# haesungpyun/seoul_tourism_recommendation_NGCF

Hardware: NVIDIA B200
Metric: ngcf_epoch_time_fwd_bwd_bpr (lower is better)
Workload: dtype f32

## Files before the change

### include/ngcf_b200.h

```cpp
#ifndef NGCF_B200_H
#define NGCF_B200_H

#include <stddef.h>
#include <stdint.h>

#ifdef __cplusplus
extern "C" {
#endif

#define NGCF_B200_ABI_VERSION 4
#define NGCF_MAX_LAYERS 8
#define NGCF_MAX_WIDTH 128
#define NGCF_ADAM_MAX_TENSORS 32

typedef enum {
    NGCF_OK = 0,
    NGCF_ERR_INVALID = -1,
    NGCF_ERR_CUDA = -2,
    NGCF_ERR_WORKSPACE = -3
} ngcf_status;

int ngcf_abi_version(void);
const char* ngcf_last_error(void);
uint64_t ngcf_launch_count(void);

int ngcf_coo_to_csr_workspace(int64_t nnz, int64_t n_rows, size_t* bytes_host);
int ngcf_coo_to_csr(const int64_t* coo_row, const int64_t* coo_col, int64_t nnz,
                    int64_t n_rows, int64_t n_cols, int transpose,
                    int32_t* rowptr ,
                    int32_t* colidx , int32_t* perm ,
                    void* workspace, size_t workspace_bytes, void* stream);

typedef struct ngcf_csr {
    int64_t n_rows;
    const int32_t* rowptr;
    const int32_t* ent;
    const int32_t* tiles;
    const int32_t* hub_of_row;
    const int32_t* hub_chunk_ptr;
    const int32_t* chunk_ptr;
    const int32_t* hub_ent;
    const int32_t* chunk_row;
    const int32_t* chunk_tiles;
    const int32_t* hub_rows;
    int32_t* hub_done;
    const uint32_t* key_l;
    const uint32_t* key_t;
    int64_t key_row_offset;
    int32_t n_tiles, n_hub, n_chunks, n_chunk_tiles;
    int32_t rowptr_nnz;
    const uint32_t* tile_hubmask;
} ngcf_csr;

int ngcf_spmm_split_threshold(void);
int ngcf_spmm_tile_rows(void);
int ngcf_spmm_tile_entries(void);

int ngcf_edge_entries(const int32_t* colidx, const float* coo_val, const int32_t* perm, const uint8_t* keep_mask,
                      int32_t* ent_out, int64_t nnz, void* stream);

int ngcf_feature_mix(float* user_w, int64_t n_user, int d,
                     const float* const* tables_host, const int* widths_host,
                     const int64_t* const* idx_host, const int64_t* u_id, int64_t batch,
                     float ratio, int32_t* winner, void* stream);

int ngcf_spmm(const ngcf_csr* csr_host, const float* X, int64_t ldx, int d,
              const float* addend, int64_t ld_add,
              const int32_t* slot, const float* gsum, int64_t ld_gsum,
              float* hub_partial,
              float drop_p, uint64_t seed, const uint64_t* seed_dev, int layer, int transposed, int64_t row_offset,
              const uint8_t* keep_bits, const int32_t* c_ent, const int32_t* c_cnt,
              float* Y, int64_t ldy, void* stream);

int ngcf_node_dropout_bits(const ngcf_csr* csr_host, float drop_p, uint64_t seed, const uint64_t* seed_dev,
                           int n_layers, int64_t row_offset, uint8_t* bits_as_L, uint8_t* bits_as_Lt, void* stream);

int ngcf_node_dropout_compact(const ngcf_csr* csr_host, float drop_p, uint64_t seed, const uint64_t* seed_dev,
                              int n_layers, int64_t row_offset,
                              int32_t* const* ent_as_L_host, int32_t* const* cnt_as_L_host,
                              int32_t* const* ent_as_Lt_host, int32_t* const* cnt_as_Lt_host, void* stream);

int ngcf_entry_keys(const ngcf_csr* csr_host, int64_t row_offset, uint32_t* key_l, uint32_t* key_t, void* stream);

int ngcf_plgraph_entries(int64_t n_user, int64_t n_item, int64_t n_edges, double alpha, uint64_t seed,
                         int64_t row0, int64_t n_rows, unsigned long long* total_dev,
                         unsigned long long* keys_or_null, int64_t capacity, void* stream);
int ngcf_build_tiles(const int32_t* rowptr, int64_t n_rows, int max_rows, int max_ent, int32_t* next_scratch,
                     int32_t* tiles_out, int64_t capacity, int32_t* count_out, void* stream);

int ngcf_exchange_flag_words(void);
int ngcf_push_rows(float* const* matrix_on_rank_host, uint32_t* const* flags_on_rank_host, uint32_t* local_state,
                   int world, int rank, int64_t row0, int64_t n_rows, int d, float* multicast_or_null, void* stream);
int ngcf_push_selected_rows(float* const* matrix_on_rank_host, uint32_t* const* flags_on_rank_host, uint32_t* local_state,
                            int world, int rank, int64_t row0, int64_t n_rows, int d,
                            const int64_t* const* lists_host, const int64_t* list_offsets_host,
                            const int64_t* list_sizes_host, int n_lists, float* multicast_or_null, void* stream);

int ngcf_pack_weights(const float* W1, const float* b1, const float* W2, const float* b2,
                      int d_in, int d_out, float* wcat , float* bias_eff ,
                      void* stream);
int ngcf_pack_weights_all(const float* const* W1_host, const float* const* b1_host, const float* const* W2_host,
                          const float* const* b2_host, const int* d_in_host, const int* d_out_host, int n_layers,
                          float* const* wcat_host, float* const* bias_host, void* stream);
int ngcf_dense_fwd(const float* S, const float* E, int64_t n_rows, int d_in, int d_out,
                   const float* wcat, const float* bias_eff, float slope,
                   const float* mess_mult, const uint32_t* mess_bits, float mess_p, uint64_t seed,
                   const uint64_t* seed_dev, int layer, int64_t row_offset, float* E_out, void* stream);

int ngcf_mess_dropout_bits(int64_t n_rows, int d_out, float mess_p, uint64_t seed, const uint64_t* seed_dev, int layer,
                           int64_t row_offset, uint32_t* bits, void* stream);

int ngcf_gather_concat(const float* const* layers_host, const int* dims_host, int n_layers_plus1,
                       const int64_t* rows, int64_t row_offset, int64_t n_out,
                       float* out, int64_t ld_out, void* stream);
int ngcf_gather_concat_sets(const float* const* layers_host, const int* dims_host, int n_layers_plus1,
                            const int64_t* const* rows_host, const int64_t* offsets_host, const int64_t* sizes_host,
                            float* const* outs_host, int n_sets, int64_t ld_out, void* stream);

int ngcf_bpr_fwd_bwd(const float* u, const float* p, const float* n, int64_t batch, int D,
                     float weight_decay, float batch_size_ctor, float reg_w_u, float reg_w_p, float reg_w_n,
                     float* loss, float* gu, float* gp, float* gn, void* stream);

int ngcf_rowgrad_scatter(const int64_t* const* rows_host, const int64_t* offsets_host,
                         const float* const* g_host, const int64_t* batch_host, int n_sets, int D,
                         int32_t* slot, float* gsum, void* stream);
int ngcf_rowgrad_normalize(const int64_t* const* rows_host, const int64_t* offsets_host,
                           const int64_t* batch_host, int n_sets, const float* const* layers_host,
                           const int* dims_host, int n_layers_plus1, const int32_t* slot, float* gsum, int D,
                           void* stream);
int ngcf_rowgrad_reset(const int64_t* const* rows_host, const int64_t* offsets_host,
                       const int64_t* batch_host, int n_sets, int32_t* slot, void* stream);

int ngcf_set_wgrad_stream(void* stream_or_null);
int ngcf_wgrad_stream_forked(void);
int ngcf_dense_bwd(const float* gE_next, const int32_t* slot, const float* gsum, int64_t ld_gsum, int col_off,
                   const float* E_out, const float* S, const float* E, int64_t n_rows, int d_in, int d_out,
                   const float* W1, const float* W2, float slope,
                   const float* mess_mult, const uint32_t* mess_bits, float mess_p, uint64_t seed,
                   const uint64_t* seed_dev, int layer, int64_t row_offset, int gh_normalized, float* gS, float* gEl,
                   float* gW1, float* gb1, float* gW2, float* gb2, float* gM_scratch, void* stream);

int ngcf_score_topk_workspace(int64_t n_users, int64_t n_items, int D, int k, size_t* bytes_host);
int ngcf_score_topk(const float* U, int64_t n_users, const float* I, int64_t n_items, int D, int k,
                    float* out_val , int64_t* out_idx ,
                    void* workspace, size_t workspace_bytes, void* stream);
int ngcf_score_topk_excluding(const float* U, int64_t n_users, const float* I, int64_t n_items, int D, int k,
                              const int64_t* excl_ptr , const int32_t* excl_idx,
                              float* out_val , int64_t* out_idx ,
                              void* workspace, size_t workspace_bytes, void* stream);

int ngcf_rank_metrics(const int64_t* topk_idx, int64_t n_users, int k, const int64_t* truth_ptr,
                      const int32_t* truth_idx, const int* Ks_host, int n_K, float* per_user, float* totals,
                      void* stream);

int ngcf_adam_step(float* const* params_host, float* const* grads_host, float* const* exp_avg_host,
                   float* const* exp_avg_sq_host, const int64_t* sizes_host, int n_tensors, double lr, double beta1,
                   double beta2, double eps, double weight_decay, int64_t step, const int64_t* step_dev,
                   int zero_grads, void* stream);

int ngcf_eval_groups(const float* u, const float* items, const int64_t* item_ids, const float* rating,
                     const int64_t* group_ptr, int64_t n_groups, int group, int D, int k_hr, int k_ndcg, float weight_decay,
                     float batch_size_ctor, float* bpr, float* hit, float* ndcg, float* rmse, float* scores,
                     float* totals, void* stream);

int ngcf_sample_negatives(const int32_t* pos_ptr, const int32_t* pos_idx, const int64_t* row_user, int64_t n_rows,
                          const int64_t* candidates, int n_candidates, int ng_ratio, uint64_t seed, int64_t* out,
                          int32_t* n_short, void* stream);

int ngcf_laplacian_entries(const int64_t* user, const int64_t* item, const float* rating, int64_t n_pairs,
                           int64_t n_user, int64_t n_item, int32_t* deg, int64_t* row, int64_t* col, float* val,
                           void* stream);

int ngcf_debug_bwd_timeline(int enable, long long* out_host);
int ngcf_debug_spmm_timeline(unsigned long long* dev_buf_or_null);
int ngcf_debug_compact_timeline(unsigned long long* dev_buf_or_null);

#ifdef __cplusplus
}
#endif
#endif
```

### seoul_tourism_recommendation_ngcf_b200/NGCF.py

```python
from __future__ import annotations

import ctypes as C
import os

import numpy as np
import torch
import torch.nn as nn

import torch.distributed as dist

from . import _lib
from .plan import LaplacianPlan, node_dropout_bits, node_dropout_compact, spmm
from .sharded import RowShards, all_gather_rows

LEAKY_SLOPE = 0.2


def _stream() -> int:
    return _lib.current_stream()


class _Ctx:
    __slots__ = ("plan", "E", "S", "dims", "vals_f", "vals_b", "mess_mult", "mess_p", "seed", "seed_dev", "masked", "drop_p", "bits_f", "bits_b", "comp_f", "comp_b", "mess_bits",
                 "rows", "offsets", "W1", "W2", "fresh_key", "node_mode", "last_partial", "fm_stream")


def _capturing() -> bool:
    return torch.cuda.is_current_stream_capturing()


def _join_feature_mix(st):
    if st.fm_stream is not None:
        torch.cuda.current_stream().wait_stream(st.fm_stream)
        st.fm_stream = None


class _Propagate(torch.autograd.Function):

    @staticmethod
    def forward(ctx, mod, st: _Ctx, n_sets, user_w, item_w, *wb):
        lib = _lib.load()
        K = mod.n_layer
        W1, b1, W2, b2 = wb[0:K], wb[K:2 * K], wb[2 * K:3 * K], wb[3 * K:4 * K]
        dev = user_w.device
        sh = mod._shard
        N = mod.n_user + mod.n_item
        r0, nloc, nv = (sh.r0, sh.rows, sh.valid) if sh is not None else (0, N, N)
        X0 = mod._packed_table()
        if mod._snapshot:
            _join_feature_mix(st)
            X0 = X0.clone()
        st.E, st.S, st.W1, st.W2 = [X0], [], list(W1), list(W2)
        side = st.plan.fwd
        st.bits_f = st.bits_b = st.comp_f = st.comp_b = None
        st.node_mode = mod._node_mode
        st.last_partial = None
        if st.drop_p > 0:
            shared = st.plan.side(True, False) is side
            node_mode = mod._node_mode if all(d % 4 == 0 for d in st.dims) or mod._node_mode == "inkernel" else "bits"
            st.node_mode = node_mode
            if node_mode == "compact":
                st.comp_f, ct = node_dropout_compact(side, st.drop_p, st.seed, st.seed_dev, K, r0, as_L=True, as_Lt=shared)
                if shared:
                    st.comp_b = ct
            elif node_mode == "bits":
                st.bits_f, bt = node_dropout_bits(side, st.drop_p, st.seed, st.seed_dev, K, r0, as_L=True, as_Lt=shared)
                if shared:
                    st.bits_b = bt
        self_uses_mess_bits = mod._mess_bits
        st.mess_bits = [None] * K
        for k in range(K):
            if self_uses_mess_bits and st.mess_mult is None and st.mess_p[k] > 0 and st.dims[k + 1] % 4 == 0:
                bits = torch.empty(nloc * ((st.dims[k + 1] + 31) // 32), dtype=torch.int32, device=dev)
                _lib.check(lib.ngcf_mess_dropout_bits(nv, st.dims[k + 1], float(st.mess_p[k]), st.seed,
                                                      _lib.ptr(st.seed_dev), k, r0, bits.data_ptr(), _stream()),
                           "mess_dropout_bits")
                st.mess_bits[k] = bits
        wcats = [torch.empty(2 * st.dims[k] * st.dims[k + 1], dtype=torch.float32, device=dev) for k in range(K)]
        biases = [torch.empty(st.dims[k + 1], dtype=torch.float32, device=dev) for k in range(K)]
        _lib.check(lib.ngcf_pack_weights_all(_lib.ptr_array(W1), _lib.ptr_array(b1), _lib.ptr_array(W2), _lib.ptr_array(b2),
                                             _lib.int_array(st.dims[:K]), _lib.int_array(st.dims[1:]), K,
                                             _lib.ptr_array(wcats), _lib.ptr_array(biases), _stream()), "pack_weights_all")
        _join_feature_mix(st)
        for k in range(K):
            d_in, d_out = st.dims[k], st.dims[k + 1]
            vals = st.vals_f[k] if st.vals_f is not None else None
            S = spmm(side, vals, st.E[k], d_in, drop_p=st.drop_p, seed=st.seed, seed_dev=st.seed_dev, layer=k,
                     row_offset=r0, keep_bits=st.bits_f,
                     compact=st.comp_f[k] if st.comp_f is not None else None)
            wcat, bias = wcats[k], biases[k]
            xkey = None
            if sh is None:
                Xn = En = torch.empty(N, d_out, dtype=torch.float32, device=dev)
            elif mod._xchg is not None and d_out % 4 == 0:
                xkey = ("E", k + 1)
                Xn = mod._xchg.matrix(xkey, sh.N_pad, d_out)
                En = Xn[r0:r0 + nloc]
            else:
                Xn = torch.empty(sh.N_pad, d_out, dtype=torch.float32, device=dev)
                En = torch.zeros(nloc, d_out, dtype=torch.float32, device=dev) if nv < nloc else \
                    torch.empty(nloc, d_out, dtype=torch.float32, device=dev)
            mm = st.mess_mult[k] if st.mess_mult is not None else None
            E_loc = st.E[k][r0:r0 + nloc]
            _lib.check(lib.ngcf_dense_fwd(S.data_ptr(), E_loc.data_ptr(), nv, d_in, d_out, wcat.data_ptr(),
                                          bias.data_ptr(), LEAKY_SLOPE, _lib.ptr(mm[r0:r0 + nloc] if mm is not None else None),
                                          _lib.ptr(st.mess_bits[k]), float(st.mess_p[k]), st.seed, _lib.ptr(st.seed_dev), k, r0, En.data_ptr(),
                                          _stream()),
                       "dense_fwd")
            if xkey is not None and k == K - 1:
                mod._xchg.push_selected(xkey, r0, nloc, st.rows[:n_sets], st.offsets[:n_sets])
                st.last_partial = xkey
            elif xkey is not None:
                mod._xchg.push(xkey, r0, nloc)
            elif sh is not None:
                all_gather_rows(Xn, En, mod._group)
            st.S.append(S)
            st.E.append(Xn)
        D = sum(st.dims)
        layers, dims = _lib.ptr_array(st.E), _lib.int_array(st.dims)
        outs = [torch.empty(st.rows[j].numel(), D, dtype=torch.float32, device=dev) for j in range(n_sets)]
        _lib.check(lib.ngcf_gather_concat_sets(layers, dims, K + 1, _lib.ptr_array(st.rows[:n_sets]),
                                               _lib.i64_array(st.offsets[:n_sets]),
                                               _lib.i64_array([r.numel() for r in st.rows[:n_sets]]), _lib.ptr_array(outs),
                                               n_sets, D, _stream()), "gather_concat_sets")
        ctx.st, ctx.mod, ctx.n_sets = st, mod, n_sets
        return tuple(outs)

    @staticmethod
    def backward(ctx, *gouts):
        lib = _lib.load()
        st, mod, n_sets = ctx.st, ctx.mod, ctx.n_sets
        mod._check_fresh(st, "loss.backward()")
        K, dims = mod.n_layer, st.dims
        dev = st.E[0].device
        sh = mod._shard
        N = mod.n_user + mod.n_item
        r0, nloc, nv, N_all = (sh.r0, sh.rows, sh.valid, sh.N_pad) if sh is not None else (0, N, N, N)
        D = sum(dims)
        g = [(go.contiguous() if go is not None else torch.zeros(st.rows[j].numel(), D, device=dev))
             for j, go in enumerate(gouts)]
        batch = [r.numel() for r in st.rows[:n_sets]]
        rows_h, offs_h = _lib.ptr_array(st.rows[:n_sets]), _lib.i64_array(st.offsets[:n_sets])
        g_h, batch_h = _lib.ptr_array(g), _lib.i64_array(batch)
        slot = mod._slot_map(N_all, dev)
        gsum = torch.empty(sum(batch), D, dtype=torch.float32, device=dev)
        _lib.check(lib.ngcf_rowgrad_scatter(rows_h, offs_h, g_h, batch_h, n_sets, D, slot.data_ptr(),
                                            gsum.data_ptr(), _stream()), "rowgrad_scatter")
        _lib.check(lib.ngcf_rowgrad_normalize(rows_h, offs_h, batch_h, n_sets, _lib.ptr_array(st.E), _lib.int_array(dims),
                                              K + 1, slot.data_ptr(), gsum.data_ptr(), D, _stream()), "rowgrad_normalize")
        slot_loc = slot[r0:r0 + nloc]
        sizes = [dims[k + 1] * dims[k] for k in range(K)]
        n_flat = 2 * sum(sizes) + 2 * sum(dims[1:])
        if sh is not None and mod._xchg is not None:
            f_pad = (n_flat + 3) // 4 * 4
            wg_all = mod._xchg.matrix(("wgrad", f_pad), sh.world, f_pad)
            flat = wg_all[sh.rank, :n_flat]
            flat.zero_()
        else:
            wg_all = None
            flat = torch.zeros(n_flat, dtype=torch.float32, device=dev)
        gW1, gW2, gb1, gb2, o = [], [], [], [], 0
        for k in range(K):
            gW1.append(flat[o:o + sizes[k]].view(dims[k + 1], dims[k])); o += sizes[k]
            gW2.append(flat[o:o + sizes[k]].view(dims[k + 1], dims[k])); o += sizes[k]
            gb1.append(flat[o:o + dims[k + 1]]); o += dims[k + 1]
            gb2.append(flat[o:o + dims[k + 1]]); o += dims[k + 1]
        side = st.plan.side(True, st.vals_b is not None)
        if st.drop_p > 0 and st.node_mode == "compact" and st.comp_b is None:
            _, st.comp_b = node_dropout_compact(side, st.drop_p, st.seed, st.seed_dev, K, r0, as_L=False, as_Lt=True)
        if st.drop_p > 0 and st.node_mode == "bits" and st.bits_b is None:
            _, st.bits_b = node_dropout_bits(side, st.drop_p, st.seed, st.seed_dev, K, r0, as_L=False, as_Lt=True)
        gE_next = None
        col_off = D
        overlap = _capturing() or (sh is not None and mod._xchg is not None)
        if overlap:
            if mod._side_stream is None:
                mod._side_stream = torch.cuda.Stream(device=dev)
            _lib.check(lib.ngcf_set_wgrad_stream(mod._side_stream.cuda_stream), "set_wgrad_stream")
            lib.ngcf_wgrad_stream_forked()
            gM_keep = []
        else:
            gM_scratch = torch.empty(nloc, max(dims[1:]), dtype=torch.float32, device=dev)
        for k in range(K - 1, -1, -1):
            d_in, d_out = dims[k], dims[k + 1]
            col_off -= d_out
            peer = sh is not None and mod._xchg is not None and d_in % 4 == 0
            if peer:
                gS_all = mod._xchg.matrix(("gS", d_in), N_all, d_in)
                gS = gS_all[r0:r0 + nloc]
            else:
                gS = torch.empty(nloc, d_in, dtype=torch.float32, device=dev)
            if peer and k == 0:
                gE0_all = mod._xchg.matrix(("gE0", d_in), N_all, d_in)
                gEl = gE0_all[r0:r0 + nloc]
            else:
                gEl = torch.empty(nloc, d_in, dtype=torch.float32, device=dev)
            mm = st.mess_mult[k] if st.mess_mult is not None else None
            if overlap:
                gM_scratch = torch.empty(nloc, dims[k + 1], dtype=torch.float32, device=dev)
                gM_keep.append(gM_scratch)
            _lib.check(lib.ngcf_dense_bwd(_lib.ptr(gE_next), slot_loc.data_ptr(), gsum.data_ptr(), D, col_off,
                                          st.E[k + 1][r0:r0 + nloc].data_ptr(), st.S[k].data_ptr(),
                                          st.E[k][r0:r0 + nloc].data_ptr(), nv, d_in, d_out,
                                          st.W1[k].data_ptr(), st.W2[k].data_ptr(), LEAKY_SLOPE,
                                          _lib.ptr(mm[r0:r0 + nloc] if mm is not None else None),
                                          _lib.ptr(st.mess_bits[k]), float(st.mess_p[k]), st.seed,
                                          _lib.ptr(st.seed_dev), k, r0, 1, gS.data_ptr(),
                                          gEl.data_ptr(),
                                          gW1[k].data_ptr(), gb1[k].data_ptr(), gW2[k].data_ptr(), gb2[k].data_ptr(),
                                          gM_scratch.data_ptr(), _stream()), "dense_bwd")
            if peer:
                mod._xchg.push(("gS", d_in), r0, nloc)
            elif sh is not None:
                gS_all = torch.empty(N_all, d_in, dtype=torch.float32, device=dev)
                all_gather_rows(gS_all, gS, mod._group)
            else:
                gS_all = gS
            vals = st.vals_b[k] if st.vals_b is not None else None
            last = (k == 0)
            gE_next = spmm(side, vals, gS_all, d_in, addend=gEl, slot=slot_loc if last else None,
                           gsum=gsum if last else None, drop_p=st.drop_p, seed=st.seed, seed_dev=st.seed_dev, layer=k,
                           transposed=True, row_offset=r0, keep_bits=st.bits_b,
                           compact=st.comp_b[k] if st.comp_b is not None else None)
            if mod._trace is not None:
                mod._trace.append(dict(k=k, gS=gS.clone(), gEl=gEl.clone(), gE=gE_next.clone()))
        if overlap:
            _lib.check(lib.ngcf_set_wgrad_stream(None), "set_wgrad_stream")
            if lib.ngcf_wgrad_stream_forked():
                torch.cuda.current_stream().wait_stream(mod._side_stream)
        _lib.check(lib.ngcf_rowgrad_reset(rows_h, offs_h, batch_h, n_sets, slot.data_ptr(), _stream()),
                   "rowgrad_reset")
        if sh is not None:
            if mod._xchg is not None and dims[0] % 4 == 0:
                mod._xchg.push(("gE0", dims[0]), r0, nloc)
                gE0 = gE0_all.clone()
            else:
                gE0 = torch.empty(N_all, dims[0], dtype=torch.float32, device=dev)
                all_gather_rows(gE0, gE_next, mod._group)
            if wg_all is not None:
                mod._xchg.push(("wgrad", wg_all.shape[1]), sh.rank, 1)
                total = wg_all.sum(0)[:n_flat]
                gW1, gW2, gb1, gb2, o = [], [], [], [], 0
                for k in range(K):
                    gW1.append(total[o:o + sizes[k]].view(dims[k + 1], dims[k])); o += sizes[k]
                    gW2.append(total[o:o + sizes[k]].view(dims[k + 1], dims[k])); o += sizes[k]
                    gb1.append(total[o:o + dims[k + 1]]); o += dims[k + 1]
                    gb2.append(total[o:o + dims[k + 1]]); o += dims[k + 1]
            else:
                dist.all_reduce(flat, group=mod._group)
        else:
            gE0 = gE_next
        gU, gI = gE0[:mod.n_user], gE0[mod.n_user:N]
        return (None, None, None, gU, gI, *gW1, *gb1, *gW2, *gb2)


class NGCF(nn.Module):

    def __init__(self, embed_size: int, layer_size: list, node_dropout: float, mess_dropout: list,
                 emb_ratio: float, lap_list: list, num_dict: dict, batch_size: int, device, *, rng: str = "device",
                 snapshot: bool = False):
        super().__init__()
        if rng not in ("device", "reference"):
            raise ValueError("rng must be 'device' or 'reference'")
        self.n_user = int(num_dict['user'])
        self.n_item = int(num_dict['item'])
        self.emb_size = int(embed_size)
        self.weight_size = list(layer_size)
        self.n_layer = len(self.weight_size)
        self.batch_size = batch_size
        self.device = device
        self.node_dropout = node_dropout
        self.mess_dropout = mess_dropout
        self.emb_ratio = emb_ratio
        self.rng = rng
        if max([self.emb_size] + self.weight_size) > 128 or self.n_layer > 8:
            raise ValueError("embedding/layer widths up to 128 and up to 8 layers are supported")

        w = self.emb_size // 5
        self.feat_widths = [w, w, w, w, self.emb_size - 4 * w]
        self.month_emb = nn.Embedding(int(num_dict['month']), w)
        self.day_emb = nn.Embedding(int(num_dict['day']), w)
        self.sex_emb = nn.Embedding(int(num_dict['sex']), w)
        self.age_emb = nn.Embedding(int(num_dict['age']), w)
        self.dow_emb = nn.Embedding(int(num_dict['dayofweek']), self.feat_widths[4])
        self.item_embedding = nn.Embedding(self.n_item, self.emb_size)
        self.user_embedding = nn.Embedding(self.n_user, self.emb_size)
        self.lap_list = lap_list
        self.set_layers()
        self._plans = {}
        self._table = None
        self._slot = None
        self._winner = None
        self._last = None
        self._all_E = None
        self._mess_bits = os.environ.get("NGCF_B200_MESS_BITS", "0") == "1"
        self._node_mode = "compact"
        self._snapshot = bool(snapshot) or os.environ.get("NGCF_B200_SNAPSHOT", "0") == "1"
        self._mix_count = 0
        self._seed_gen = None
        self._seed_dev = None
        self._shard = None
        self._group = None
        self._xchg = None
        self._side_stream = None
        self._side_stream3 = None
        self._trace = None
        self._inject = None

    def set_layers(self):
        init = nn.init.kaiming_uniform_
        init(self.user_embedding.weight)
        init(self.item_embedding.weight)
        init(self.age_emb.weight)
        init(self.sex_emb.weight)
        init(self.month_emb.weight)
        init(self.dow_emb.weight)
        init(self.day_emb.weight)
        sizes = [self.emb_size] + self.weight_size
        w1, w2, nd, md = [], [], [], []
        for k in range(self.n_layer):
            w1.append(nn.Linear(sizes[k], sizes[k + 1], bias=True))
            w2.append(nn.Linear(sizes[k], sizes[k + 1], bias=True))
            if self.node_dropout is not None:
                nd.append(nn.Dropout(p=self.node_dropout))
            if self.mess_dropout is not None:
                md.append(nn.Dropout(p=self.mess_dropout[k]))
        self.w1_list = nn.Sequential(*w1)
        self.w2_list = nn.Sequential(*w2)
        self.node_dropout_list = nn.Sequential(*nd)
        self.mess_dropout_list = nn.Sequential(*md)

    def shard(self, group=None, shards=None):
        if not dist.is_initialized():
            raise RuntimeError("NGCF.shard() needs an initialised torch.distributed process group")
        if self.rng != "device":
            raise ValueError("row-sharded runs need rng='device' (masks are keyed on global coordinates in-kernel)")
        world, rank = dist.get_world_size(group), dist.get_rank(group)
        self._shard = shards if shards is not None else RowShards(self.n_user + self.n_item, world, rank)
        if self._shard.N != self.n_user + self.n_item or self._shard.world != world or self._shard.rank != rank:
            raise ValueError("the shard descriptor does not match this model / process group")
        self._group = group
        self._plans, self._table, self._slot = {}, None, None
        self._xchg = None
        if world > 1 and os.environ.get("NGCF_B200_EXCHANGE", "peer") != "nccl":
            try:
                from .sharded import PeerExchange
                self._xchg = PeerExchange(group, self.user_embedding.weight.device)
            except Exception as e:
                self._xchg_error = f"{type(e).__name__}: {e}"
                ok = torch.tensor([0], device=self.user_embedding.weight.device)
            else:
                ok = torch.tensor([1], device=self.user_embedding.weight.device)
            dist.all_reduce(ok, op=dist.ReduceOp.MIN, group=group)
            if int(ok) == 0:
                self._xchg = None
        if self._xchg is None and world > 1 and not getattr(self._shard, "equal", True):
            raise RuntimeError("unequal row blocks (BalancedShards) need the peer-memory exchange, which is not available "
                               "here: " + getattr(self, "_xchg_error", "disabled by NGCF_B200_EXCHANGE=nccl"))
        return self

    def exchange_description(self) -> str:
        if self._shard is None:
            return "single GPU"
        if self._xchg is not None:
            how = "NVLS multicast stores (multimem.st)" if self._xchg.multicast() else "peer-memory stores"
            return (f"contiguous row blocks; per-layer exchange of E / gS / table-gradient rows by {how} over NVLink "
                    "(ngcf_push_rows on symmetric memory, no NCCL collective anywhere in the step; the last layer's "
                    "output travels for the batch rows only; W/b gradients: one more push + a rank-ordered sum)")
        return "equal row blocks, per-layer NCCL all-gather of E / gS, all-reduce of W/b grads"

    def _packed_table(self) -> torch.Tensor:
        u, i = self.user_embedding.weight, self.item_embedding.weight
        d = self.emb_size
        adjacent = (u.is_contiguous() and i.is_contiguous() and u.dtype == torch.float32 and
                    u.data_ptr() + self.n_user * d * 4 == i.data_ptr() and
                    getattr(self, "_table", None) is not None and self._table.data_ptr() == u.data_ptr())
        if not adjacent:
            n_rows = self._shard.N_pad if self._shard is not None else self.n_user + self.n_item
            table = torch.zeros(n_rows, d, dtype=torch.float32, device=u.device)
            table[:self.n_user].copy_(u.data)
            table[self.n_user:self.n_user + self.n_item].copy_(i.data)
            u.data = table[:self.n_user]
            i.data = table[self.n_user:self.n_user + self.n_item]
            self._table = table
        return self._table if self._shard is None else self._table

    def _slot_map(self, N, dev):
        if self._slot is None or self._slot.device != dev or self._slot.numel() != N:
            self._slot = torch.full((N,), -1, dtype=torch.int32, device=dev)
        return self._slot

    def _plan(self, year_idx: int, dev) -> LaplacianPlan:
        L = self.lap_list[year_idx]
        p = self._plans.get(year_idx)
        if p is None or p.src is not L or p.coo_val.device != dev:
            p = LaplacianPlan(L, dev, shard=self._shard)
            self._plans[year_idx] = p
        return p

    def _reference_node_masks(self, nnz: int, dev):
        alive = np.arange(nnz)
        out = []
        for _ in range(self.n_layer):
            m = nn.Dropout(self.node_dropout)(torch.tensor(np.ones(alive.size))).type(torch.bool).numpy()
            alive = alive[m]
            full = np.zeros(nnz, dtype=np.uint8)
            full[alive] = 1
            out.append(torch.from_numpy(full).to(dev))
        return out

    @_lib.on_device
    def forward(self, year, u_id, age, sex, month, day, dow, pos_item, neg_item, node_flag):
        lib = _lib.load()
        dev = self.user_embedding.weight.device
        if dev.type != "cuda":
            raise RuntimeError("NGCF (B200) runs on a CUDA device only; there is no CPU fallback. "
                               "Move the module with .to('cuda').")
        K, N = self.n_layer, self.n_user + self.n_item
        if (self._side_stream is None or self._side_stream.device != dev) and not _capturing():
            self._side_stream, self._side_stream3 = (torch.cuda.Stream(device=dev) for _ in range(2))

        def ix(t):
            return t.to(device=dev, dtype=torch.int64).contiguous()

        u_id, pos_item = ix(u_id), ix(pos_item)
        feats_idx = [ix(age), ix(sex), ix(month), ix(day), ix(dow)]
        has_neg = len(neg_item) > 0
        neg_item = ix(neg_item) if has_neg else None
        year_idx = int(year.min()) % 18

        table = self._packed_table()
        if self._winner is None or self._winner.device != dev or self._winner.numel() != self.n_user:
            self._winner = torch.full((self.n_user,), -1, dtype=torch.int32, device=dev)
        tabs = [self.age_emb.weight, self.sex_emb.weight, self.month_emb.weight, self.day_emb.weight, self.dow_emb.weight]
        def mix():
            _lib.check(lib.ngcf_feature_mix(table.data_ptr(), self.n_user, self.emb_size, _lib.ptr_array(tabs),
                                            _lib.int_array(self.feat_widths), _lib.ptr_array(feats_idx), u_id.data_ptr(),
                                            u_id.numel(), float(self.emb_ratio), self._winner.data_ptr(), _stream()),
                       "feature_mix")

        fm_stream = None
        if self._shard is None and _capturing() and bool(node_flag) and \
                (self.node_dropout or 0) > 0 and self.rng == "device":
            main = torch.cuda.current_stream()
            if self._side_stream3 is None:
                self._side_stream3 = torch.cuda.Stream(device=dev)
            self._side_stream3.wait_stream(main)
            with torch.cuda.stream(self._side_stream3):
                mix()
            fm_stream = self._side_stream3
        else:
            mix()

        self._mix_count += 1
        st = _Ctx()
        st.fm_stream = fm_stream
        st.fresh_key = self._fresh_key()
        st.plan = plan = self._plan(year_idx, dev)
        if self._shard is not None and "edge_keep" in (self._inject or {}):
            raise ValueError("explicit edge masks are not supported in row-sharded mode")
        if plan.N != N:
            raise ValueError(f"Laplacian is {plan.N}x{plan.N} but n_user+n_item = {N}")
        st.dims = [self.emb_size] + self.weight_size
        inj = self._inject or {}
        st.masked = bool(node_flag) and (self.node_dropout is not None) and \
            (self.node_dropout > 0 or "edge_keep" in inj)
        st.vals_f = st.vals_b = None
        st.drop_p = 0.0
        masks = None
        if st.masked:
            if "edge_keep" in inj:
                masks = [m.to(device=dev, dtype=torch.uint8).contiguous() for m in inj["edge_keep"]]
            elif self.rng == "reference":
                masks = self._reference_node_masks(plan.nnz, dev)
            else:
                st.drop_p = float(self.node_dropout)
        st.mess_mult = None
        st.mess_p = [0.0] * K
        if "mess_mult" in inj:
            st.mess_mult = [m.to(device=dev, dtype=torch.float32).contiguous() for m in inj["mess_mult"]]
        elif self.training and self.mess_dropout is not None:
            st.mess_p = [float(p) for p in self.mess_dropout[:K]]
        need_seed = st.drop_p > 0 or any(p > 0 for p in st.mess_p)
        if not need_seed:
            st.seed = 0
        elif self.rng == "reference":
            if self._seed_gen is None:
                self._seed_gen = torch.Generator().manual_seed(torch.initial_seed() & (2 ** 63 - 1))
            st.seed = int(torch.randint(0, 2 ** 62, (1,), generator=self._seed_gen).item())
        else:
            st.seed = int(torch.randint(0, 2 ** 62, (1,)).item())
        st.seed_dev = self._seed_dev if need_seed else None
        if masks is not None:
            st.vals_f = [plan.entries(plan.fwd, masks[k]) for k in range(K)]
            st.vals_b = [plan.entries(plan.bwd, masks[k]) for k in range(K)]
        st.rows = [u_id, pos_item] + ([neg_item] if has_neg else [])
        st.offsets = [0, self.n_user] + ([self.n_user] if has_neg else [])

        wb = [l.weight for l in self.w1_list] + [l.bias for l in self.w1_list] + \
             [l.weight for l in self.w2_list] + [l.bias for l in self.w2_list]
        outs = _Propagate.apply(self, st, len(st.rows), self.user_embedding.weight, self.item_embedding.weight, *wb)
        self._last, self._all_E = st, None
        u_embeddings, pos_i_embeddings = outs[0], outs[1]
        neg_i_embeddings = outs[2] if has_neg else torch.empty(0)
        return u_embeddings, pos_i_embeddings, neg_i_embeddings

    def _fresh_key(self):
        return (self._mix_count, _lib.param_epoch(), self.user_embedding.weight._version,
                self.item_embedding.weight._version)

    def _check_fresh(self, st, what: str):
        if self._snapshot or st.fresh_key == self._fresh_key():
            return
        why = "the step that produced it also ran the optimizer" if st.fresh_key is None else \
            "another forward (feature mix) or an optimizer step ran since"
        raise RuntimeError(f"NGCF (B200): {what} needs the embedding table as the forward left it, but {why}. "
                           "Run the forward again, or construct the module with snapshot=True to keep a per-forward "
                           "copy like the reference's torch.cat (NGCF.py:120).")

    @_lib.on_device
    def _materialize(self):
        if self._last is None:
            raise AttributeError("all_users_emb / all_items_emb exist after the first forward (NGCF.py:148-149)")
        if self._all_E is None:
            self._check_fresh(self._last, "all_users_emb / all_items_emb")
            if self._last.last_partial is not None:
                sh = self._shard
                self._xchg.push(self._last.last_partial, sh.r0, sh.rows)
                self._last.last_partial = None
            st, lib = self._last, _lib.load()
            N, D = self.n_user + self.n_item, sum(st.dims)
            out = torch.empty(N, D, dtype=torch.float32, device=st.E[0].device)
            _lib.check(lib.ngcf_gather_concat(_lib.ptr_array(st.E), _lib.int_array(st.dims), self.n_layer + 1, None, 0,
                                              N, out.data_ptr(), D, _stream()), "gather_concat")
            self._all_E = out
        return self._all_E

    @property
    def all_users_emb(self):
        return self._materialize()[:self.n_user, :]

    @property
    def all_items_emb(self):
        return self._materialize()[self.n_user:, :]
```

### seoul_tourism_recommendation_ngcf_b200/_lib.py

```python
from __future__ import annotations

import ctypes as C
import os

_PKG = os.path.dirname(os.path.abspath(__file__))
LIB_PATH = os.environ.get("NGCF_B200_LIB") or os.path.join(_PKG, "libngcf_b200.so")

_vp, _i64, _i32, _f32, _u64, _sz = C.c_void_p, C.c_int64, C.c_int32, C.c_float, C.c_uint64, C.c_size_t



class NgcfCsr(C.Structure):
    _fields_ = [("n_rows", _i64), ("rowptr", _vp), ("ent", _vp), ("tiles", _vp),
                ("hub_of_row", _vp), ("hub_chunk_ptr", _vp), ("chunk_ptr", _vp), ("hub_ent", _vp),
                ("chunk_row", _vp), ("chunk_tiles", _vp), ("hub_rows", _vp), ("hub_done", _vp), ("key_l", _vp), ("key_t", _vp), ("key_row_offset", _i64),
                ("n_tiles", _i32), ("n_hub", _i32), ("n_chunks", _i32),
                ("n_chunk_tiles", _i32), ("rowptr_nnz", _i32), ("tile_hubmask", _vp)]


_csr_p = C.POINTER(NgcfCsr)

SIGNATURES = {
    "ngcf_abi_version": [],
    "ngcf_last_error": [],
    "ngcf_launch_count": [],
    "ngcf_coo_to_csr_workspace": [_i64, _i64, C.POINTER(_sz)],
    "ngcf_coo_to_csr": [_vp, _vp, _i64, _i64, _i64, C.c_int, _vp, _vp, _vp, _vp, _sz, _vp],
    "ngcf_edge_entries": [_vp, _vp, _vp, _vp, _vp, _i64, _vp],
    "ngcf_spmm_tile_rows": [],
    "ngcf_spmm_tile_entries": [],
    "ngcf_feature_mix": [_vp, _i64, C.c_int, C.POINTER(_vp), C.POINTER(C.c_int), C.POINTER(_vp), _vp, _i64, _f32,
                         _vp, _vp],
    "ngcf_spmm_split_threshold": [],
    "ngcf_spmm": [_csr_p, _vp, _i64, C.c_int, _vp, _i64, _vp, _vp, _i64, _vp, _f32, _u64, _vp, C.c_int, C.c_int, _i64,
                  _vp, _vp, _vp, _vp, _i64, _vp],
    "ngcf_entry_keys": [_csr_p, _i64, _vp, _vp, _vp],
    "ngcf_node_dropout_compact": [_csr_p, _f32, _u64, _vp, C.c_int, _i64, C.POINTER(_vp), C.POINTER(_vp), C.POINTER(_vp),
                                  C.POINTER(_vp), _vp],
    "ngcf_node_dropout_bits": [_csr_p, _f32, _u64, _vp, C.c_int, _i64, _vp, _vp, _vp],
    "ngcf_pack_weights": [_vp, _vp, _vp, _vp, C.c_int, C.c_int, _vp, _vp, _vp],
    "ngcf_pack_weights_all": [C.POINTER(_vp), C.POINTER(_vp), C.POINTER(_vp), C.POINTER(_vp), C.POINTER(C.c_int),
                              C.POINTER(C.c_int), C.c_int, C.POINTER(_vp), C.POINTER(_vp), _vp],
    "ngcf_dense_fwd": [_vp, _vp, _i64, C.c_int, C.c_int, _vp, _vp, _f32, _vp, _vp, _f32, _u64, _vp, C.c_int, _i64, _vp,
                       _vp],
    "ngcf_mess_dropout_bits": [_i64, C.c_int, _f32, _u64, _vp, C.c_int, _i64, _vp, _vp],
    "ngcf_gather_concat": [C.POINTER(_vp), C.POINTER(C.c_int), C.c_int, _vp, _i64, _i64, _vp, _i64, _vp],
    "ngcf_gather_concat_sets": [C.POINTER(_vp), C.POINTER(C.c_int), C.c_int, C.POINTER(_vp), C.POINTER(_i64), C.POINTER(_i64),
                                C.POINTER(_vp), C.c_int, _i64, _vp],
    "ngcf_bpr_fwd_bwd": [_vp, _vp, _vp, _i64, C.c_int, _f32, _f32, _f32, _f32, _f32, _vp, _vp, _vp, _vp, _vp],
    "ngcf_rowgrad_scatter": [C.POINTER(_vp), C.POINTER(_i64), C.POINTER(_vp), C.POINTER(_i64), C.c_int, C.c_int, _vp,
                             _vp, _vp],
    "ngcf_rowgrad_reset": [C.POINTER(_vp), C.POINTER(_i64), C.POINTER(_i64), C.c_int, _vp, _vp],
    "ngcf_dense_bwd": [_vp, _vp, _vp, _i64, C.c_int, _vp, _vp, _vp, _i64, C.c_int, C.c_int, _vp, _vp, _f32, _vp, _vp, _f32,
                       _u64, _vp, C.c_int, _i64, C.c_int, _vp, _vp, _vp, _vp, _vp, _vp, _vp, _vp],
    "ngcf_set_wgrad_stream": [_vp],
    "ngcf_wgrad_stream_forked": [],
    "ngcf_rowgrad_normalize": [C.POINTER(_vp), C.POINTER(_i64), C.POINTER(_i64), C.c_int, C.POINTER(_vp),
                               C.POINTER(C.c_int), C.c_int, _vp, _vp, C.c_int, _vp],
    "ngcf_adam_step": [C.POINTER(_vp), C.POINTER(_vp), C.POINTER(_vp), C.POINTER(_vp), C.POINTER(_i64), C.c_int,
                       C.c_double, C.c_double, C.c_double, C.c_double, C.c_double, _i64, _vp, C.c_int, _vp],
    "ngcf_debug_bwd_timeline": [C.c_int, _vp],
    "ngcf_debug_spmm_timeline": [_vp],
    "ngcf_debug_compact_timeline": [_vp],
    "ngcf_score_topk_workspace": [_i64, _i64, C.c_int, C.c_int, C.POINTER(_sz)],
    "ngcf_eval_groups": [_vp, _vp, _vp, _vp, _vp, _i64, C.c_int, C.c_int, C.c_int, C.c_int, _f32, _f32, _vp, _vp, _vp, _vp, _vp,
                         _vp, _vp],
    "ngcf_sample_negatives": [_vp, _vp, _vp, _i64, _vp, C.c_int, C.c_int, _u64, _vp, _vp, _vp],
    "ngcf_laplacian_entries": [_vp, _vp, _vp, _i64, _i64, _i64, _vp, _vp, _vp, _vp, _vp],
    "ngcf_plgraph_entries": [_i64, _i64, _i64, C.c_double, _u64, _i64, _i64, _vp, _vp, _i64, _vp],
    "ngcf_build_tiles": [_vp, _i64, C.c_int, C.c_int, _vp, _vp, _i64, _vp, _vp],
    "ngcf_exchange_flag_words": [],
    "ngcf_push_rows": [C.POINTER(_vp), C.POINTER(_vp), _vp, C.c_int, C.c_int, _i64, _i64, C.c_int, _vp, _vp],
    "ngcf_push_selected_rows": [C.POINTER(_vp), C.POINTER(_vp), _vp, C.c_int, C.c_int, _i64, _i64, C.c_int, C.POINTER(_vp),
                                C.POINTER(_i64), C.POINTER(_i64), C.c_int, _vp, _vp],
    "ngcf_score_topk": [_vp, _i64, _vp, _i64, C.c_int, C.c_int, _vp, _vp, _vp, _sz, _vp],
    "ngcf_score_topk_excluding": [_vp, _i64, _vp, _i64, C.c_int, C.c_int, _vp, _vp, _vp, _vp, _vp, _sz, _vp],
    "ngcf_rank_metrics": [_vp, _i64, C.c_int, _vp, _vp, C.POINTER(C.c_int), C.c_int, _vp, _vp, _vp],
}

_lib = None


def load() -> C.CDLL:
    global _lib
    if _lib is not None:
        return _lib
    if not os.path.exists(LIB_PATH):
        raise RuntimeError(
            f"{LIB_PATH} is missing: the NGCF B200 hot path has no CPU/PyTorch fallback. "
            "Build it with `python -m seoul_tourism_recommendation_ngcf_b200.build` (needs nvcc, targets sm_100a).")
    lib = C.CDLL(LIB_PATH)
    for name, argtypes in SIGNATURES.items():
        fn = getattr(lib, name)
        fn.argtypes = argtypes
        fn.restype = {"ngcf_last_error": C.c_char_p, "ngcf_launch_count": C.c_uint64}.get(name, C.c_int)
    _lib = lib
    return lib


def check(rc: int, what: str = "") -> None:
    if rc != 0:
        msg = load().ngcf_last_error()
        raise RuntimeError(f"ngcf_b200 {what} failed (status {rc}): {msg.decode() if msg else '?'}")


def ptr(t) -> int | None:
    return None if t is None else t.data_ptr()


def ptr_array(tensors):
    return (_vp * len(tensors))(*[None if t is None else t.data_ptr() for t in tensors])


def ptr_array_int(addrs):
    return (_vp * len(addrs))(*[int(a) for a in addrs])


def int_array(vals):
    return (C.c_int * len(vals))(*[int(v) for v in vals])


def i64_array(vals):
    return (_i64 * len(vals))(*[int(v) for v in vals])


_param_epoch = 0


def bump_param_epoch() -> None:
    global _param_epoch
    _param_epoch += 1


def param_epoch() -> int:
    return _param_epoch


def on_device(fn):
    import functools

    import torch

    @functools.wraps(fn)
    def wrapped(*args, **kwargs):
        dev = None
        for a in list(args) + list(kwargs.values()):
            if isinstance(a, torch.Tensor):
                if a.device.type == "cuda":
                    dev = a.device
                    break
            elif isinstance(a, torch.nn.Module):
                q = next(a.parameters(), None)
                if q is not None and q.device.type == "cuda":
                    dev = q.device
                    break
        if dev is None or dev.index is None or dev.index == torch.cuda.current_device():
            return fn(*args, **kwargs)
        with torch.cuda.device(dev):
            return fn(*args, **kwargs)
    return wrapped


def current_stream() -> int:
    import torch
    try:
        return torch._C._cuda_getCurrentRawStream(torch._C._cuda_getDevice())
    except AttributeError:
        return torch.cuda.current_stream().cuda_stream
```

### seoul_tourism_recommendation_ngcf_b200/csrc/dense.cu

```cuda
#include "common.cuh"

namespace {

__global__ void pack_weights_kernel(const float* __restrict__ W1, const float* __restrict__ b1,
                                    const float* __restrict__ W2, const float* __restrict__ b2, int d_in, int d_out,
                                    float* __restrict__ wcat, float* __restrict__ bias_eff) {
    const int total = 2 * d_in * d_out;
    for (int i = blockIdx.x * blockDim.x + threadIdx.x; i < total; i += gridDim.x * blockDim.x) {
        const int k = i / d_out, o = i % d_out;
        wcat[i] = k < d_in ? W1[o * d_in + k] : W2[o * d_in + (k - d_in)];
    }
    for (int o = blockIdx.x * blockDim.x + threadIdx.x; o < d_out; o += gridDim.x * blockDim.x)
        bias_eff[o] = 2.0f * b1[o] + b2[o];
}

struct PackAllArgs {
    const float* W1[NGCF_MAX_LAYERS];
    const float* b1[NGCF_MAX_LAYERS];
    const float* W2[NGCF_MAX_LAYERS];
    const float* b2[NGCF_MAX_LAYERS];
    float* wcat[NGCF_MAX_LAYERS];
    float* bias[NGCF_MAX_LAYERS];
    int d_in[NGCF_MAX_LAYERS], d_out[NGCF_MAX_LAYERS];
};
__global__ void pack_weights_all_kernel(PackAllArgs a) {
    const int l = blockIdx.y, d_in = a.d_in[l], d_out = a.d_out[l];
    const float* __restrict__ W1 = a.W1[l];
    const float* __restrict__ W2 = a.W2[l];
    const int total = 2 * d_in * d_out;
    for (int i = blockIdx.x * blockDim.x + threadIdx.x; i < total; i += gridDim.x * blockDim.x) {
        const int k = i / d_out, o = i % d_out;
        a.wcat[l][i] = k < d_in ? W1[o * d_in + k] : W2[o * d_in + (k - d_in)];
    }
    for (int o = blockIdx.x * blockDim.x + threadIdx.x; o < d_out; o += gridDim.x * blockDim.x)
        a.bias[l][o] = 2.0f * a.b1[l][o] + a.b2[l][o];
}

constexpr int FWD_R = 64;
constexpr int FWD_THREADS = 256;

struct FwdArgs {
    const float* S;
    const float* E;
    int64_t n_rows;
    int d_in, d_out;
    const float* wcat;
    const float* bias_eff;
    float slope;
    const float* mess_mult;
    const uint32_t* mess_bits;
    float mess_p;
    uint64_t seed;
    const uint64_t* seed_dev;
    int layer;
    float* E_out;
    int KP;
    int n_tiles;
    int64_t row_off;
};

template <int NCG>
__global__ void __launch_bounds__(FWD_THREADS) dense_fwd_kernel(FwdArgs a) {
    extern __shared__ __align__(16) float smem[];
    constexpr int NP = 64 * NCG;
    const int KP = a.KP, XLD = KP + 4;
    float* Ws = smem;
    float* Xs = Ws + (size_t)KP * NP;
    float* Bs = Xs + (size_t)FWD_R * XLD;
    const int tid = threadIdx.x, tx = tid & 15, ty = tid >> 4;
    const int d_in = a.d_in, d_out = a.d_out, K = 2 * d_in;
    const uint64_t seed = a.mess_p > 0.f ? ngcf_seed(a.seed, a.seed_dev) : 0ull;

    for (int i = tid; i < KP * NP; i += FWD_THREADS) {
        const int k = i / NP, o = i % NP;
        Ws[i] = (k < K && o < d_out) ? a.wcat[k * d_out + o] : 0.f;
    }
    for (int o = tid; o < NP; o += FWD_THREADS) Bs[o] = o < d_out ? a.bias_eff[o] : 0.f;

    const bool vec_in = (d_in % 4 == 0);
    const bool vec_out = (d_out % 4 == 0);
    for (int tile = blockIdx.x; tile < a.n_tiles; tile += gridDim.x) {
        const int64_t row0 = (int64_t)tile * FWD_R;
        __syncthreads();
        if (vec_in) {
            const int d4 = d_in / 4;
            for (int i = tid; i < FWD_R * d4; i += FWD_THREADS) {
                const int r = i / d4, c = (i % d4) * 4;
                const int64_t row = row0 + r;
                float4 s = make_float4(0.f, 0.f, 0.f, 0.f), e = s;
                if (row < a.n_rows) {
                    s = ld_f4(a.S + row * d_in + c);
                    e = ld_f4(a.E + row * d_in + c);
                }
                st_f4(Xs + r * XLD + c, make_float4(s.x + e.x, s.y + e.y, s.z + e.z, s.w + e.w));
                st_f4(Xs + r * XLD + d_in + c, make_float4(s.x * e.x, s.y * e.y, s.z * e.z, s.w * e.w));
            }
        } else {
            for (int i = tid; i < FWD_R * d_in; i += FWD_THREADS) {
                const int r = i / d_in, c = i % d_in;
                const int64_t row = row0 + r;
                float s = 0.f, e = 0.f;
                if (row < a.n_rows) {
                    s = a.S[row * d_in + c];
                    e = a.E[row * d_in + c];
                }
                Xs[r * XLD + c] = s + e;
                Xs[r * XLD + d_in + c] = s * e;
            }
        }
        if (KP > K) {
            for (int i = tid; i < FWD_R * (KP - K); i += FWD_THREADS) {
                const int r = i / (KP - K), c = K + i % (KP - K);
                Xs[r * XLD + c] = 0.f;
            }
        }
        __syncthreads();

        float acc[NCG][4][4];
#pragma unroll
        for (int g = 0; g < NCG; ++g)
#pragma unroll
            for (int r = 0; r < 4; ++r)
#pragma unroll
                for (int c = 0; c < 4; ++c) acc[g][r][c] = 0.f;

        for (int k = 0; k < KP; k += 4) {
            float4 av[4];
#pragma unroll
            for (int r = 0; r < 4; ++r) av[r] = ld_f4(Xs + (ty * 4 + r) * XLD + k);
#pragma unroll
            for (int kk = 0; kk < 4; ++kk) {
#pragma unroll
                for (int g = 0; g < NCG; ++g) {
                    const float4 b = ld_f4(Ws + (k + kk) * NP + g * 64 + tx * 4);
#pragma unroll
                    for (int r = 0; r < 4; ++r) {
                        const float x = kk == 0 ? av[r].x : kk == 1 ? av[r].y : kk == 2 ? av[r].z : av[r].w;
                        acc[g][r][0] = fmaf(x, b.x, acc[g][r][0]);
                        acc[g][r][1] = fmaf(x, b.y, acc[g][r][1]);
                        acc[g][r][2] = fmaf(x, b.z, acc[g][r][2]);
                        acc[g][r][3] = fmaf(x, b.w, acc[g][r][3]);
                    }
                }
            }
        }

#pragma unroll
        for (int r = 0; r < 4; ++r) {
            const int64_t row = row0 + ty * 4 + r;
            if (row >= a.n_rows) continue;
#pragma unroll
            for (int g = 0; g < NCG; ++g) {
                const int c0 = g * 64 + tx * 4;
                if (c0 >= d_out) continue;
                float o[4];
#pragma unroll
                for (int c = 0; c < 4; ++c) {
                    float m = acc[g][r][c] + Bs[c0 + c];
                    float v = m > 0.f ? m : a.slope * m;
                    const int col = c0 + c;
                    if (col < d_out) {
                        if (a.mess_mult) v *= a.mess_mult[row * d_out + col];
                        else if (a.mess_bits) v *= mess_multiplier_bits(a.mess_bits, a.mess_p, row, d_out, col);
                        else if (a.mess_p > 0.f) v *= mess_multiplier(a.mess_p, seed, a.layer, (uint64_t)((row + a.row_off) * d_out + col));
                    }
                    o[c] = v;
                }
                if (vec_out) {
                    st_f4(a.E_out + row * d_out + c0, make_float4(o[0], o[1], o[2], o[3]));
                } else {
#pragma unroll
                    for (int c = 0; c < 4; ++c)
                        if (c0 + c < d_out) a.E_out[row * d_out + c0 + c] = o[c];
                }
            }
        }
    }
}

struct BwdArgs {
    const float* gE_next;
    const int32_t* slot;
    const float* gsum;
    int64_t ld_gsum;
    int col_off;
    const float* E_out;
    const float* S;
    const float* E;
    int64_t n_rows;
    int d_in, d_out;
    const float* W1;
    const float* W2;
    float slope;
    const float* mess_mult;
    const uint32_t* mess_bits;
    float mess_p;
    uint64_t seed;
    const uint64_t* seed_dev;
    int layer;
    float* gS;
    float* gEl;
    float* gW1;
    float* gb1;
    float* gW2;
    float* gb2;
    int n_tiles;
    int64_t row_off;
    int gh_normalized;
};

template <int DC, int R, int THREADS>
__global__ void __launch_bounds__(THREADS) dense_bwd_kernel(BwdArgs a) {
    constexpr int TX = DC / 4;
    constexpr int TY = THREADS / TX;
    constexpr int RPT = R / TY;
    constexpr int OB = (DC / 4) / TY;
    constexpr int LD = DC + 4;
    constexpr int NW = THREADS / 32;
    constexpr int QN = DC / 32;
    static_assert(R % TY == 0 && (DC / 4) % TY == 0 && R % NW == 0, "tile shape");

    extern __shared__ __align__(16) float smem[];
    float* W1s = smem;
    float* W2s = W1s + DC * DC;
    float* GM = W2s + DC * DC;
    float* Ss = GM + R * LD;
    float* Es = Ss + R * LD;
    float* CS = Es + R * LD;

    const int tid = threadIdx.x, lane = tid & 31, warp = tid >> 5;
    const int tx = tid % TX, ty = tid / TX;
    const int d_in = a.d_in, d_out = a.d_out;
    const uint64_t seed = a.mess_p > 0.f ? ngcf_seed(a.seed, a.seed_dev) : 0ull;

    for (int i = tid; i < DC * DC; i += THREADS) {
        const int o = i / DC, j = i % DC;
        const bool in = (o < d_out && j < d_in);
        W1s[i] = in ? a.W1[o * d_in + j] : 0.f;
        W2s[i] = in ? a.W2[o * d_in + j] : 0.f;
    }

    float accW1[OB][4][4], accW2[OB][4][4];
#pragma unroll
    for (int q = 0; q < OB; ++q)
#pragma unroll
        for (int o = 0; o < 4; ++o)
#pragma unroll
            for (int j = 0; j < 4; ++j) accW1[q][o][j] = accW2[q][o][j] = 0.f;
    float colsum[QN];
#pragma unroll
    for (int q = 0; q < QN; ++q) colsum[q] = 0.f;

    const bool vec_in = (d_in % 4 == 0);
    const int KO = (d_out + 3) & ~3;

    for (int tile = blockIdx.x; tile < a.n_tiles; tile += gridDim.x) {
        const int64_t row0 = (int64_t)tile * R;
        __syncthreads();
        for (int r = warp; r < R; r += NW) {
            const int64_t row = row0 + r;
            float e[QN], gm[QN];
            float nrm2 = 0.f;
#pragma unroll
            for (int q = 0; q < QN; ++q) {
                const int c = lane + 32 * q;
                e[q] = (row < a.n_rows && c < d_out) ? a.E_out[row * d_out + c] : 0.f;
                nrm2 = fmaf(e[q], e[q], nrm2);
            }
            nrm2 = warp_sum(nrm2);
            const float n = fmaxf(sqrtf(nrm2), 1e-12f);
            const int s = (row < a.n_rows && a.slot) ? a.slot[row] : -1;
            float gh[QN];
            float dot = 0.f;
#pragma unroll
            for (int q = 0; q < QN; ++q) {
                const int c = lane + 32 * q;
                gh[q] = (s >= 0 && c < d_out) ? a.gsum[(int64_t)s * a.ld_gsum + a.col_off + c] : 0.f;
                dot = fmaf(e[q], gh[q], dot);
            }
            if (s >= 0) dot = warp_sum(dot) / n;
#pragma unroll
            for (int q = 0; q < QN; ++q) {
                const int c = lane + 32 * q;
                float g = 0.f;
                if (row < a.n_rows && c < d_out) {
                    g = a.gE_next ? a.gE_next[row * d_out + c] : 0.f;
                    if (s >= 0) g += a.gh_normalized ? gh[q] : (gh[q] - (e[q] / n) * dot) / n;
                    float mult = 1.f;
                    if (a.mess_mult) mult = a.mess_mult[row * d_out + c];
                    else if (a.mess_bits) mult = mess_multiplier_bits(a.mess_bits, a.mess_p, row, d_out, c);
                    else if (a.mess_p > 0.f) mult = mess_multiplier(a.mess_p, seed, a.layer, (uint64_t)((row + a.row_off) * d_out + c));
                    g *= mult * (e[q] > 0.f ? 1.f : a.slope);
                }
                gm[q] = g;
                colsum[q] += g;
                if (c < DC) GM[r * LD + c] = g;
            }
        }
        if (vec_in) {
            const int d4 = d_in / 4;
            for (int i = tid; i < R * (DC / 4); i += THREADS) {
                const int r = i / (DC / 4), c4 = i % (DC / 4);
                const int64_t row = row0 + r;
                float4 s = make_float4(0.f, 0.f, 0.f, 0.f), e = s;
                if (row < a.n_rows && c4 < d4) {
                    s = ld_f4(a.S + row * d_in + c4 * 4);
                    e = ld_f4(a.E + row * d_in + c4 * 4);
                }
                st_f4(Ss + r * LD + c4 * 4, s);
                st_f4(Es + r * LD + c4 * 4, e);
            }
        } else {
            for (int i = tid; i < R * DC; i += THREADS) {
                const int r = i / DC, c = i % DC;
                const int64_t row = row0 + r;
                const bool in = (row < a.n_rows && c < d_in);
                Ss[r * LD + c] = in ? a.S[row * d_in + c] : 0.f;
                Es[r * LD + c] = in ? a.E[row * d_in + c] : 0.f;
            }
        }
        __syncthreads();

        {
            float t1[RPT][4], t2[RPT][4];
#pragma unroll
            for (int r = 0; r < RPT; ++r)
#pragma unroll
                for (int c = 0; c < 4; ++c) t1[r][c] = t2[r][c] = 0.f;
            for (int k = 0; k < KO; k += 4) {
                float4 av[RPT];
#pragma unroll
                for (int r = 0; r < RPT; ++r) av[r] = ld_f4(GM + (ty * RPT + r) * LD + k);
#pragma unroll
                for (int kk = 0; kk < 4; ++kk) {
                    const float4 b1 = ld_f4(W1s + (k + kk) * DC + tx * 4);
                    const float4 b2 = ld_f4(W2s + (k + kk) * DC + tx * 4);
#pragma unroll
                    for (int r = 0; r < RPT; ++r) {
                        const float x = kk == 0 ? av[r].x : kk == 1 ? av[r].y : kk == 2 ? av[r].z : av[r].w;
                        t1[r][0] = fmaf(x, b1.x, t1[r][0]); t1[r][1] = fmaf(x, b1.y, t1[r][1]);
                        t1[r][2] = fmaf(x, b1.z, t1[r][2]); t1[r][3] = fmaf(x, b1.w, t1[r][3]);
                        t2[r][0] = fmaf(x, b2.x, t2[r][0]); t2[r][1] = fmaf(x, b2.y, t2[r][1]);
                        t2[r][2] = fmaf(x, b2.z, t2[r][2]); t2[r][3] = fmaf(x, b2.w, t2[r][3]);
                    }
                }
            }
            const int j0 = tx * 4;
#pragma unroll
            for (int r = 0; r < RPT; ++r) {
                const int rr = ty * RPT + r;
                const int64_t row = row0 + rr;
                if (row >= a.n_rows || j0 >= d_in) continue;
                const float4 e4 = ld_f4(Es + rr * LD + j0), s4 = ld_f4(Ss + rr * LD + j0);
                float gs[4] = {fmaf(t2[r][0], e4.x, t1[r][0]), fmaf(t2[r][1], e4.y, t1[r][1]),
                               fmaf(t2[r][2], e4.z, t1[r][2]), fmaf(t2[r][3], e4.w, t1[r][3])};
                float ge[4] = {fmaf(t2[r][0], s4.x, t1[r][0]), fmaf(t2[r][1], s4.y, t1[r][1]),
                               fmaf(t2[r][2], s4.z, t1[r][2]), fmaf(t2[r][3], s4.w, t1[r][3])};
                if (vec_in) {
                    st_f4(a.gS + row * d_in + j0, make_float4(gs[0], gs[1], gs[2], gs[3]));
                    st_f4(a.gEl + row * d_in + j0, make_float4(ge[0], ge[1], ge[2], ge[3]));
                } else {
#pragma unroll
                    for (int c = 0; c < 4; ++c)
                        if (j0 + c < d_in) {
                            a.gS[row * d_in + j0 + c] = gs[c];
                            a.gEl[row * d_in + j0 + c] = ge[c];
                        }
                }
            }
        }

        for (int r = 0; r < R; ++r) {
            const float4 s4 = ld_f4(Ss + r * LD + tx * 4), e4 = ld_f4(Es + r * LD + tx * 4);
            const float x1[4] = {s4.x + e4.x, s4.y + e4.y, s4.z + e4.z, s4.w + e4.w};
            const float x2[4] = {s4.x * e4.x, s4.y * e4.y, s4.z * e4.z, s4.w * e4.w};
#pragma unroll
            for (int q = 0; q < OB; ++q) {
                const float4 g4 = ld_f4(GM + r * LD + (ty + TY * q) * 4);
                const float g[4] = {g4.x, g4.y, g4.z, g4.w};
#pragma unroll
                for (int o = 0; o < 4; ++o)
#pragma unroll
                    for (int j = 0; j < 4; ++j) {
                        accW1[q][o][j] = fmaf(g[o], x1[j], accW1[q][o][j]);
                        accW2[q][o][j] = fmaf(g[o], x2[j], accW2[q][o][j]);
                    }
            }
        }
    }

#pragma unroll
    for (int q = 0; q < OB; ++q)
#pragma unroll
        for (int o = 0; o < 4; ++o) {
            const int oo = (ty + TY * q) * 4 + o;
            if (oo >= d_out) continue;
#pragma unroll
            for (int j = 0; j < 4; ++j) {
                const int jj = tx * 4 + j;
                if (jj < d_in) {
                    atomicAdd(a.gW1 + oo * d_in + jj, accW1[q][o][j]);
                    atomicAdd(a.gW2 + oo * d_in + jj, accW2[q][o][j]);
                }
            }
        }
    __syncthreads();
#pragma unroll
    for (int q = 0; q < QN; ++q) CS[warp * DC + lane + 32 * q] = colsum[q];
    __syncthreads();
    for (int c = tid; c < d_out; c += THREADS) {
        float s = 0.f;
        for (int w = 0; w < NW; ++w) s += CS[w * DC + c];
        atomicAdd(a.gb2 + c, s);
        atomicAdd(a.gb1 + c, 2.0f * s);
    }
}

template <typename K>
int set_smem(K kernel, size_t bytes) {
    if (bytes > 48 * 1024) {
        cudaError_t e = cudaFuncSetAttribute(kernel, cudaFuncAttributeMaxDynamicSharedMemorySize, (int)bytes);
        if (e != cudaSuccess) {
            ngcf_set_error("cudaFuncSetAttribute(%zu bytes smem) failed: %s", bytes, cudaGetErrorString(e));
            return NGCF_ERR_CUDA;
        }
    }
    return NGCF_OK;
}

inline bool aligned16(const void* p) { return (reinterpret_cast<uintptr_t>(p) & 15) == 0; }

}

bool ngcf_dense_fwd_tc_eligible(int d_in, int d_out);
int ngcf_dense_fwd_tc(const float* S, const float* E, int64_t n_rows, int d_in, int d_out, const float* wcat,
                      const float* bias_eff, float slope, const float* mess_mult, const uint32_t* mess_bits, float mess_p,
                      uint64_t seed,
                      const uint64_t* seed_dev, int layer, int64_t row_offset, float* E_out, cudaStream_t st);

bool ngcf_dense_bwd_tc_eligible(int d_in, int d_out, int gh_normalized);
int ngcf_dense_bwd_tc(const float* gE_next, const int32_t* slot, const float* gsum, int64_t ld_gsum, int col_off,
                      const float* E_out, const float* S, const float* E, int64_t n_rows, int d_in, int d_out,
                      const float* W1, const float* W2, float slope, const float* mess_mult, const uint32_t* mess_bits,
                      float mess_p,
                      uint64_t seed, const uint64_t* seed_dev, int layer, int64_t row_offset, int gh_normalized, float* gS, float* gEl,
                      float* gW1, float* gb1, float* gW2, float* gb2, float* gM_scratch, cudaStream_t st);

extern "C" int ngcf_pack_weights(const float* W1, const float* b1, const float* W2, const float* b2, int d_in,
                                 int d_out, float* wcat, float* bias_eff, void* stream) {
    NGCF_REQUIRE(W1 && b1 && W2 && b2 && wcat && bias_eff, "pack_weights: null pointer");
    NGCF_REQUIRE(d_in > 0 && d_in <= NGCF_MAX_WIDTH && d_out > 0 && d_out <= NGCF_MAX_WIDTH,
                 "pack_weights: widths %d -> %d not in [1,%d]", d_in, d_out, NGCF_MAX_WIDTH);
    pack_weights_kernel<<<32, 256, 0, as_stream(stream)>>>(W1, b1, W2, b2, d_in, d_out, wcat, bias_eff);
    NGCF_LAUNCH_OK("pack_weights_kernel");
    return NGCF_OK;
}

extern "C" int ngcf_pack_weights_all(const float* const* W1_host, const float* const* b1_host, const float* const* W2_host,
                                     const float* const* b2_host, const int* d_in_host, const int* d_out_host, int n_layers,
                                     float* const* wcat_host, float* const* bias_host, void* stream) {
    NGCF_REQUIRE(W1_host && b1_host && W2_host && b2_host && d_in_host && d_out_host && wcat_host && bias_host,
                 "pack_weights_all: null pointer");
    NGCF_REQUIRE(n_layers >= 1 && n_layers <= NGCF_MAX_LAYERS, "pack_weights_all: %d layers", n_layers);
    PackAllArgs a{};
    for (int l = 0; l < n_layers; ++l) {
        NGCF_REQUIRE(W1_host[l] && b1_host[l] && W2_host[l] && b2_host[l] && wcat_host[l] && bias_host[l],
                     "pack_weights_all: null pointer (layer %d)", l);
        NGCF_REQUIRE(d_in_host[l] > 0 && d_in_host[l] <= NGCF_MAX_WIDTH && d_out_host[l] > 0 && d_out_host[l] <= NGCF_MAX_WIDTH,
                     "pack_weights_all: widths %d -> %d not in [1,%d]", d_in_host[l], d_out_host[l], NGCF_MAX_WIDTH);
        a.W1[l] = W1_host[l]; a.b1[l] = b1_host[l]; a.W2[l] = W2_host[l]; a.b2[l] = b2_host[l];
        a.wcat[l] = wcat_host[l]; a.bias[l] = bias_host[l]; a.d_in[l] = d_in_host[l]; a.d_out[l] = d_out_host[l];
    }
    pack_weights_all_kernel<<<dim3(32, (unsigned)n_layers), 256, 0, as_stream(stream)>>>(a);
    NGCF_LAUNCH_OK("pack_weights_all_kernel");
    return NGCF_OK;
}

extern "C" int ngcf_dense_fwd(const float* S, const float* E, int64_t n_rows, int d_in, int d_out, const float* wcat,
                              const float* bias_eff, float slope, const float* mess_mult, const uint32_t* mess_bits, float mess_p,
                      uint64_t seed,
                              const uint64_t* seed_dev, int layer, int64_t row_offset, float* E_out, void* stream) {
    NGCF_REQUIRE(S && E && wcat && bias_eff && E_out, "dense_fwd: null pointer");
    NGCF_REQUIRE(d_in > 0 && d_in <= NGCF_MAX_WIDTH && d_out > 0 && d_out <= NGCF_MAX_WIDTH,
                 "dense_fwd: widths %d -> %d not in [1,%d]", d_in, d_out, NGCF_MAX_WIDTH);
    NGCF_REQUIRE(mess_p >= 0.f && mess_p < 1.f, "dense_fwd: mess_p %f not in [0,1)", mess_p);
    NGCF_REQUIRE(n_rows >= 0 && n_rows < ((int64_t)1 << 31), "dense_fwd: n_rows %lld", (long long)n_rows);
    if (n_rows == 0) return NGCF_OK;
    if (ngcf_dense_fwd_tc_eligible(d_in, d_out) && aligned16(S) && aligned16(E) &&
        aligned16(E_out) && (!mess_mult || aligned16(mess_mult)))
        return ngcf_dense_fwd_tc(S, E, n_rows, d_in, d_out, wcat, bias_eff, slope, mess_mult, mess_bits, mess_p, seed, seed_dev,
                                 layer, row_offset, E_out, as_stream(stream));
    FwdArgs a{S, E, n_rows, d_in, d_out, wcat, bias_eff, slope, mess_mult, mess_bits, mess_p, seed, seed_dev, layer, E_out,
              (2 * d_in + 3) & ~3, (int)ceil_div64(n_rows, FWD_R), row_offset};
    const int ncg = d_out <= 64 ? 1 : 2;
    const size_t smem = sizeof(float) * ((size_t)a.KP * 64 * ncg + (size_t)FWD_R * (a.KP + 4) + 64 * ncg);
    const int per_sm = smem > 110 * 1024 ? 1 : (smem > 72 * 1024 ? 2 : 3);
    const int grid = (int)min((int64_t)a.n_tiles, (int64_t)ngcf_num_sms() * per_sm);
    int rc;
    if (ncg == 1) {
        if ((rc = set_smem(dense_fwd_kernel<1>, smem)) != NGCF_OK) return rc;
        dense_fwd_kernel<1><<<grid, FWD_THREADS, smem, as_stream(stream)>>>(a);
    } else {
        if ((rc = set_smem(dense_fwd_kernel<2>, smem)) != NGCF_OK) return rc;
        dense_fwd_kernel<2><<<grid, FWD_THREADS, smem, as_stream(stream)>>>(a);
    }
    NGCF_LAUNCH_OK("dense_fwd_kernel");
    return NGCF_OK;
}

extern "C" int ngcf_dense_bwd(const float* gE_next, const int32_t* slot, const float* gsum, int64_t ld_gsum,
                              int col_off, const float* E_out, const float* S, const float* E, int64_t n_rows,
                              int d_in, int d_out, const float* W1, const float* W2, float slope,
                              const float* mess_mult, const uint32_t* mess_bits, float mess_p, uint64_t seed,
                              const uint64_t* seed_dev, int layer, int64_t row_offset, int gh_normalized, float* gS,
                              float* gEl, float* gW1, float* gb1, float* gW2, float* gb2, float* gM_scratch, void* stream) {
    NGCF_REQUIRE(E_out && S && E && W1 && W2 && gS && gEl && gW1 && gb1 && gW2 && gb2, "dense_bwd: null pointer");
    NGCF_REQUIRE(!slot || gsum, "dense_bwd: slot given without gsum");
    NGCF_REQUIRE(d_in > 0 && d_in <= NGCF_MAX_WIDTH && d_out > 0 && d_out <= NGCF_MAX_WIDTH,
                 "dense_bwd: widths %d -> %d not in [1,%d]", d_in, d_out, NGCF_MAX_WIDTH);
    NGCF_REQUIRE(mess_p >= 0.f && mess_p < 1.f, "dense_bwd: mess_p %f not in [0,1)", mess_p);
    NGCF_REQUIRE(n_rows >= 0 && n_rows < ((int64_t)1 << 31), "dense_bwd: n_rows %lld", (long long)n_rows);
    if (n_rows == 0) return NGCF_OK;
    if (gM_scratch && ngcf_dense_bwd_tc_eligible(d_in, d_out, gh_normalized) && aligned16(S) &&
        aligned16(E) && aligned16(gS) && aligned16(gEl) && aligned16(gM_scratch))
        return ngcf_dense_bwd_tc(gE_next, slot, gsum, ld_gsum, col_off, E_out, S, E, n_rows, d_in, d_out, W1, W2,
                                 slope, mess_mult, mess_bits, mess_p, seed, seed_dev, layer, row_offset, gh_normalized, gS,
                                 gEl, gW1, gb1, gW2, gb2, gM_scratch, as_stream(stream));
    BwdArgs a{gE_next, slot, gsum, ld_gsum, col_off, E_out, S, E, n_rows, d_in, d_out, W1, W2, slope, mess_mult,
              mess_bits, mess_p, seed, seed_dev, layer, gS, gEl, gW1, gb1, gW2, gb2, 0, row_offset, gh_normalized};
    int rc;
    if (d_in <= 64 && d_out <= 64) {
        constexpr int DC = 64, R = 64, T = 256;
        a.n_tiles = (int)ceil_div64(n_rows, R);
        const size_t smem = sizeof(float) * (2 * DC * DC + 3 * R * (DC + 4) + (T / 32) * DC);
        const int grid = (int)min((int64_t)a.n_tiles, (int64_t)ngcf_num_sms() * 2);
        if ((rc = set_smem(dense_bwd_kernel<DC, R, T>, smem)) != NGCF_OK) return rc;
        dense_bwd_kernel<DC, R, T><<<grid, T, smem, as_stream(stream)>>>(a);
    } else {
        constexpr int DC = 128, R = 32, T = 512;
        a.n_tiles = (int)ceil_div64(n_rows, R);
        const size_t smem = sizeof(float) * (2 * DC * DC + 3 * R * (DC + 4) + (T / 32) * DC);
        const int grid = (int)min((int64_t)a.n_tiles, (int64_t)ngcf_num_sms());
        if ((rc = set_smem(dense_bwd_kernel<DC, R, T>, smem)) != NGCF_OK) return rc;
        dense_bwd_kernel<DC, R, T><<<grid, T, smem, as_stream(stream)>>>(a);
    }
    NGCF_LAUNCH_OK("dense_bwd_kernel");
    return NGCF_OK;
}

namespace {
__global__ void mess_bits_kernel(int64_t n_rows, int d_out, int words, float p, uint64_t seed0, const uint64_t* seed_dev,
                                 int layer, int64_t row_off, uint32_t* __restrict__ bits) {
    const int64_t i = blockIdx.x * (int64_t)blockDim.x + threadIdx.x;
    if (i >= n_rows * words) return;
    const int64_t row = i / words;
    const int w = (int)(i % words);
    const uint64_t seed = ngcf_seed(seed0, seed_dev);
    uint32_t out = 0;
#pragma unroll
    for (int q = 0; q < 8; ++q) {
        const int col = w * 32 + q * 4;
        if (col < d_out) {
            const float4 m = mess_multiplier4(p, seed, layer, (uint64_t)((row + row_off) * d_out + col) >> 2);
            out |= (m.x != 0.f ? 1u : 0u) << (q * 4) | (m.y != 0.f ? 2u : 0u) << (q * 4) | (m.z != 0.f ? 4u : 0u) << (q * 4) |
                   (m.w != 0.f ? 8u : 0u) << (q * 4);
        }
    }
    bits[i] = out;
}
}

extern "C" int ngcf_mess_dropout_bits(int64_t n_rows, int d_out, float mess_p, uint64_t seed, const uint64_t* seed_dev,
                                      int layer, int64_t row_offset, uint32_t* bits, void* stream) {
    NGCF_REQUIRE(bits && n_rows >= 0, "mess_dropout_bits: null pointer");
    NGCF_REQUIRE(d_out > 0 && d_out <= NGCF_MAX_WIDTH && d_out % 4 == 0, "mess_dropout_bits: width %d", d_out);
    NGCF_REQUIRE(mess_p > 0.f && mess_p < 1.f, "mess_dropout_bits: mess_p %f not in (0,1)", mess_p);
    if (n_rows == 0) return NGCF_OK;
    const int words = (d_out + 31) / 32;
    mess_bits_kernel<<<(unsigned)ceil_div64(n_rows * words, 256), 256, 0, as_stream(stream)>>>(
        n_rows, d_out, words, mess_p, seed, seed_dev, layer, row_offset, bits);
    NGCF_LAUNCH_OK("mess_bits_kernel");
    return NGCF_OK;
}
```

### seoul_tourism_recommendation_ngcf_b200/csrc/dense_tc.cu

```cuda
#include <stdlib.h>

#include "tc.cuh"
#include "tmap.h"

namespace {

using namespace tc;

__device__ long long g_bwd_dbg[4][8][8];
__device__ int g_bwd_dbg_on = 0;
#define BWD_STAMP(role, it, k)                                                   \
    do {                                                                         \
        if (dbg && lane == 0 && (it) < 8) g_bwd_dbg[role][it][k] = clock64();    \
    } while (0)

constexpr int TC_ROWS = 128;
constexpr int TC_EPI_WARPS = 4;
constexpr int TC_LOAD_WARPS = 8;
constexpr int TC_THREADS = (TC_EPI_WARPS + 1 + TC_LOAD_WARPS) * 32;
constexpr int TC_MAX_KB = 4;
constexpr int TC_A_BLOCK = TC_ROWS * 128;

struct FwdTcArgs {
    const float* S;
    const float* E;
    int64_t n_rows;
    int d_in, d_out;
    const float* wcat;
    const float* bias_eff;
    float slope;
    const float* mess_mult;
    const uint32_t* mess_bits;
    float mess_p;
    uint64_t seed;
    const uint64_t* seed_dev;
    int layer;
    float* E_out;
    int n_tiles;
    int64_t row_off;
    int64_t ld_in;
    int in_off, w_row1, w_row2, out_off, d_out_full, mode;
};
enum { FW_SINGLE = 0, FW_PARTIAL = 1, FW_FINAL = 2 };

constexpr int FW_EPI_WARPS = 8;
constexpr int FW_MMA_WARP = FW_EPI_WARPS;

__device__ __forceinline__ int stage_off(int r, int c) { return r * 32 + ((c ^ (r & 7)) << 2); }

enum { MM_NONE = 0, MM_MULT = 1, MM_BITS = 2, MM_HASH = 3 };
static inline int mess_mode(const float* mess_mult, const uint32_t* mess_bits, float mess_p) {
    return mess_mult ? MM_MULT : (mess_p > 0.f ? (mess_bits ? MM_BITS : MM_HASH) : MM_NONE);
}

template <int MM>
__device__ __forceinline__ void fwd_epilogue_role(const FwdTcArgs& a, float* stage, const float* bias_s, uint64_t* tmem_full,
                                                  uint64_t* tmem_empty, uint32_t tmem_base, int n_my, int warp, int lane,
                                                  bool dbg) {
    const int d_out = a.d_out;
    const uint64_t seed = MM == MM_HASH ? ngcf_seed(a.seed, a.seed_dev) : 0ull;
    const uint32_t thr = ngcf_threshold16(a.mess_p);
    float* st = stage + warp * 32 * 32;
    const int quarter = warp & 3, c = warp >> 2;
    const int rr = lane >> 3, c4 = lane & 7;
    const bool has_chunk = c * 32 < d_out;
    const float inv_keep = 1.0f / (1.0f - a.mess_p);
    for (int it = 0; it < n_my; ++it) {
        const int tile = blockIdx.x + it * gridDim.x;
        const int buf = it & 1;
        BWD_STAMP(0, it, 0);
        mbar_wait(&tmem_full[buf], (it >> 1) & 1);
        BWD_STAMP(0, it, 1);
        tc_fence_after_sync();
        float v[32];
        if (has_chunk) tmem_ld_32x32(tmem_base + ((uint32_t)(quarter * 32) << 16) + buf * 64 + c * 32, v);
        tc_fence_before_sync();
        __syncwarp();
        if (lane == 0) mbar_arrive(&tmem_empty[buf]);
        BWD_STAMP(0, it, 3);
        if (!has_chunk) continue;
        const int64_t row_base = (int64_t)tile * TC_ROWS + quarter * 32;
#pragma unroll
        for (int j = 0; j < 32; j += 4)
            st_f4(st + stage_off(lane, j >> 2), make_float4(v[j], v[j + 1], v[j + 2], v[j + 3]));
        __syncwarp();
        float4 r4[8];
#pragma unroll
        for (int i = 0; i < 8; ++i) r4[i] = ld_f4(st + stage_off(i * 4 + rr, c4));
        __syncwarp();
        BWD_STAMP(0, it, 4);
        const int col = c * 32 + c4 * 4;
        if (col < d_out) {
            const int gcol = a.out_off + col;
            const float4 b4 = *reinterpret_cast<const float4*>(bias_s + col);
            const int words = (a.d_out_full + 31) >> 5;
#pragma unroll
            for (int i = 0; i < 8; ++i) {
                const int64_t row = row_base + i * 4 + rr;
                if (row >= a.n_rows) continue;
                float* dst = a.E_out + row * a.d_out_full + gcol;
                float4 x = r4[i];
                if (a.mode == FW_PARTIAL) {
                    st_f4(dst, x);
                    continue;
                }
                if (a.mode == FW_FINAL) {
                    const float4 prev = ld_f4(dst);
                    x.x += prev.x; x.y += prev.y; x.z += prev.z; x.w += prev.w;
                }
                x.x += b4.x; x.y += b4.y; x.z += b4.z; x.w += b4.w;
                x.x = x.x > 0.f ? x.x : a.slope * x.x;
                x.y = x.y > 0.f ? x.y : a.slope * x.y;
                x.z = x.z > 0.f ? x.z : a.slope * x.z;
                x.w = x.w > 0.f ? x.w : a.slope * x.w;
                if (MM == MM_BITS) {
                    const uint32_t w = a.mess_bits[row * words + (gcol >> 5)] >> (gcol & 31);
                    x.x = w & 1u ? x.x * inv_keep : 0.f; x.y = w & 2u ? x.y * inv_keep : 0.f;
                    x.z = w & 4u ? x.z * inv_keep : 0.f; x.w = w & 8u ? x.w * inv_keep : 0.f;
                } else if (MM == MM_HASH) {
                    const float4 mm = mess_multiplier4_pre(thr, inv_keep, seed, a.layer,
                                                           (uint64_t)((row + a.row_off) * a.d_out_full + gcol) >> 2);
                    x.x *= mm.x; x.y *= mm.y; x.z *= mm.z; x.w *= mm.w;
                } else if (MM == MM_MULT) {
                    const float4 mm = ld_f4(a.mess_mult + row * a.d_out_full + gcol);
                    x.x *= mm.x; x.y *= mm.y; x.z *= mm.z; x.w *= mm.w;
                }
                st_f4(dst, x);
            }
        }
        BWD_STAMP(0, it, 2);
    }
}

constexpr int F2_CONV_WARPS = 4;
constexpr int F2_TMA_WARP = FW_EPI_WARPS + 1;
constexpr int F2_THREADS = (FW_EPI_WARPS + 2 + F2_CONV_WARPS) * 32;
constexpr int F2_RAW_STAGES = 2;
constexpr int F2_A_SLOTS = 2;
constexpr int F2_RAW_BYTES = 2 * TC_A_BLOCK;

struct FwdTmaArgs {
    FwdTcArgs b;
    alignas(64) CUtensorMap tmS;
    alignas(64) CUtensorMap tmE;
};

struct Bars2 {
    uint64_t raw_full[F2_RAW_STAGES], raw_empty[F2_RAW_STAGES];
    uint64_t a_full[F2_A_SLOTS], a_empty[F2_A_SLOTS];
    uint64_t tmem_full[2], tmem_empty[2];
    uint64_t b_ready;
    uint32_t tmem_base;
};

template <int MM>
__global__ void __launch_bounds__(F2_THREADS, 1) dense_fwd_tma_kernel(const __grid_constant__ FwdTmaArgs p) {
    extern __shared__ uint8_t smem_raw[];
    const FwdTcArgs& a = p.b;
    const uint32_t base = (smem_u32(smem_raw) + 1023u) & ~1023u;
    uint8_t* smem = smem_raw + (base - smem_u32(smem_raw));
    const int d_in = a.d_in, d_out = a.d_out;
    const int KBH = d_in / 32, KB = 2 * KBH;
    const int b_block = d_out * 128;
    uint8_t* RAW = smem;
    uint8_t* AOP = RAW + F2_RAW_STAGES * F2_RAW_BYTES;
    uint8_t* B_hi = AOP + F2_A_SLOTS * 2 * TC_A_BLOCK;
    uint8_t* B_lo = B_hi + KB * b_block;
    float* bias_s = reinterpret_cast<float*>(B_lo + KB * b_block);
    float* stage = bias_s + 64;
    Bars2* bars = reinterpret_cast<Bars2*>(stage + FW_EPI_WARPS * 32 * 32);

    const int tid = threadIdx.x, warp = tid >> 5, lane = tid & 31;
    pdl_launch_dependents();
    if (tid == 0) {
        for (int i = 0; i < F2_RAW_STAGES; ++i) {
            mbar_init(&bars->raw_full[i], 1);
            mbar_init(&bars->raw_empty[i], F2_CONV_WARPS);
        }
        for (int i = 0; i < F2_A_SLOTS; ++i) {
            mbar_init(&bars->a_full[i], F2_CONV_WARPS);
            mbar_init(&bars->a_empty[i], 1);
        }
        for (int i = 0; i < 2; ++i) {
            mbar_init(&bars->tmem_full[i], 1);
            mbar_init(&bars->tmem_empty[i], FW_EPI_WARPS);
        }
        mbar_init(&bars->b_ready, FW_EPI_WARPS);
        fence_mbar_init();
        tma_prefetch_desc(&p.tmS);
        tma_prefetch_desc(&p.tmE);
    }
    if (warp == FW_MMA_WARP) tmem_alloc(&bars->tmem_base, 128);
    tc_fence_before_sync();
    __syncthreads();
    tc_fence_after_sync();
    const uint32_t tmem_base = bars->tmem_base;
    const int n_my = (a.n_tiles - (int)blockIdx.x + (int)gridDim.x - 1) / (int)gridDim.x;
    const int n_q = n_my * KBH;
    const bool dbg = g_bwd_dbg_on == 1 && blockIdx.x == 0 && (warp == 0 || warp >= FW_MMA_WARP);
    if (dbg && lane == 0 && warp == 0) g_bwd_dbg[0][7][7] = clock64();
    pdl_wait();
    if (dbg && lane == 0 && warp == 0) g_bwd_dbg[0][7][6] = clock64();

    if (warp < FW_EPI_WARPS) {
        constexpr int ET = FW_EPI_WARPS * 32;
        constexpr int WMAX = 64 * TC_MAX_KB * 8 / ET;
        float4 wv[WMAX];
        const int n_items = d_out * KB * 8;
#pragma unroll
        for (int q = 0; q < WMAX; ++q) {
            const int i = q * ET + tid;
            wv[q] = make_float4(0.f, 0.f, 0.f, 0.f);
            if (i < n_items) {
                const int n = i % d_out, c = (i / d_out) & 7, kb = i / (d_out * 8);
                const int k = kb * 32 + c * 4;
                const int wrow = k < d_in ? a.w_row1 + k : a.w_row2 + (k - d_in);
                const float* src = a.wcat + (int64_t)wrow * a.d_out_full + a.out_off + n;
                wv[q] = make_float4(src[0], src[a.d_out_full], src[2 * a.d_out_full], src[3 * a.d_out_full]);
            }
        }
#pragma unroll
        for (int q = 0; q < WMAX; ++q) {
            const int i = q * ET + tid;
            if (i < n_items) {
                const int n = i % d_out, c = (i / d_out) & 7, kb = i / (d_out * 8);
                float4 hi, lo;
                split_tf32(wv[q], hi, lo);
                const uint32_t off = kb * b_block + sw128_offset(n, c);
                *reinterpret_cast<float4*>(B_hi + off) = hi;
                *reinterpret_cast<float4*>(B_lo + off) = lo;
            }
        }
        for (int i = tid; i < 64; i += ET) bias_s[i] = i < d_out ? a.bias_eff[a.out_off + i] : 0.f;
        fence_proxy_async_smem();
        asm volatile("bar.sync 1, %0;" ::"n"(ET) : "memory");
        if (lane == 0) mbar_arrive(&bars->b_ready);
        if (dbg && lane == 0) g_bwd_dbg[0][7][5] = clock64();
        fwd_epilogue_role<MM>(a, stage, bias_s, bars->tmem_full, bars->tmem_empty, tmem_base, n_my, warp, lane, dbg);
    } else if (warp == FW_MMA_WARP) {
        const uint32_t idesc = umma_idesc_tf32(TC_ROWS, d_out, 0, 0);
        int j = 0;
        mbar_wait(&bars->b_ready, 0);
        for (int it = 0; it < n_my; ++it) {
            const int buf = it & 1;
            mbar_wait(&bars->tmem_empty[buf], ((it >> 1) & 1) ^ 1);
            BWD_STAMP(1, it, 0);
            tc_fence_after_sync();
            const uint32_t tmem_d = tmem_base + buf * 64;
            uint32_t accumulate = 0;
            for (int hh = 0; hh < KBH; ++hh)
                for (int part = 0; part < 2; ++part, ++j) {
                    const int slot = j % F2_A_SLOTS;
                    mbar_wait(&bars->a_full[slot], (j / F2_A_SLOTS) & 1);
                    BWD_STAMP(1, it, 1 + hh * 2 + part);
                    tc_fence_after_sync();
                    if (lane == 0) {
                        const int kb = part * KBH + hh;
                        const uint32_t a_hi = smem_u32(AOP + slot * 2 * TC_A_BLOCK), a_lo = a_hi + TC_A_BLOCK;
                        const uint32_t b_hi = smem_u32(B_hi + kb * b_block), b_lo = smem_u32(B_lo + kb * b_block);
#pragma unroll
                        for (int k = 0; k < 4; ++k) {
                            const uint64_t dah = umma_desc_sw128(a_hi + k * 32, 16, 1024);
                            const uint64_t dal = umma_desc_sw128(a_lo + k * 32, 16, 1024);
                            const uint64_t dbh = umma_desc_sw128(b_hi + k * 32, 16, 1024);
                            const uint64_t dbl = umma_desc_sw128(b_lo + k * 32, 16, 1024);
                            umma_tf32(tmem_d, dah, dbh, idesc, accumulate);
                            umma_tf32(tmem_d, dal, dbh, idesc, 1);
                            umma_tf32(tmem_d, dah, dbl, idesc, 1);
                            accumulate = 1;
                        }
                        umma_commit(&bars->a_empty[slot]);
                    }
                    __syncwarp();
                }
            if (lane == 0) umma_commit(&bars->tmem_full[buf]);
            __syncwarp();
        }
    } else if (warp == F2_TMA_WARP) {
        if (lane == 0) {
            for (int q = 0; q < n_q; ++q) {
                const int it = q / KBH, hh = q % KBH, s = q % F2_RAW_STAGES;
                const int tile = blockIdx.x + it * gridDim.x;
                mbar_wait(&bars->raw_empty[s], ((q / F2_RAW_STAGES) & 1) ^ 1);
                BWD_STAMP(3, it, hh);
                mbar_expect_tx(&bars->raw_full[s], F2_RAW_BYTES);
                const uint32_t dst = smem_u32(RAW + s * F2_RAW_BYTES);
                tma_load_2d(dst, &p.tmS, a.in_off + hh * 32, tile * TC_ROWS, &bars->raw_full[s]);
                tma_load_2d(dst + TC_A_BLOCK, &p.tmE, a.in_off + hh * 32, tile * TC_ROWS, &bars->raw_full[s]);
            }
        }
    } else {
        const int lt = tid - (FW_EPI_WARPS + 2) * 32;
        constexpr int LT = F2_CONV_WARPS * 32;
        constexpr int NQ = TC_A_BLOCK / 16 / LT;
        int j = 0;
        for (int q = 0; q < n_q; ++q, j += 2) {
            const int s = q % F2_RAW_STAGES;
            mbar_wait(&bars->raw_full[s], (q / F2_RAW_STAGES) & 1);
            if (dbg && lane == 0 && warp == F2_TMA_WARP + 1 && q / KBH < 8) g_bwd_dbg[2][q / KBH][(q % KBH) * 3] = clock64();
            const uint8_t* rs = RAW + s * F2_RAW_BYTES;
            float4 sv[NQ], ev[NQ];
#pragma unroll
            for (int i = 0; i < NQ; ++i) {
                const uint32_t off = (uint32_t)(i * LT + lt) * 16u;
                sv[i] = *reinterpret_cast<const float4*>(rs + off);
                ev[i] = *reinterpret_cast<const float4*>(rs + TC_A_BLOCK + off);
            }
            {
                const int slot = j % F2_A_SLOTS;
                mbar_wait(&bars->a_empty[slot], ((j / F2_A_SLOTS) & 1) ^ 1);
                if (dbg && lane == 0 && warp == F2_TMA_WARP + 1 && q / KBH < 8) g_bwd_dbg[2][q / KBH][(q % KBH) * 3 + 1] = clock64();
                uint8_t* hi_p = AOP + slot * 2 * TC_A_BLOCK;
#pragma unroll
                for (int i = 0; i < NQ; ++i) {
                    const uint32_t off = (uint32_t)(i * LT + lt) * 16u;
                    const float4 x = make_float4(sv[i].x + ev[i].x, sv[i].y + ev[i].y, sv[i].z + ev[i].z, sv[i].w + ev[i].w);
                    float4 hi, lo;
                    split_tf32_trunc(x, hi, lo);
                    *reinterpret_cast<float4*>(hi_p + off) = hi;
                    *reinterpret_cast<float4*>(hi_p + TC_A_BLOCK + off) = lo;
                }
                fence_proxy_async_smem();
                __syncwarp();
                if (lane == 0) {
                    mbar_arrive(&bars->raw_empty[s]);
                    mbar_arrive(&bars->a_full[slot]);
                }
            }
            {
                const int slot = (j + 1) % F2_A_SLOTS;
                mbar_wait(&bars->a_empty[slot], (((j + 1) / F2_A_SLOTS) & 1) ^ 1);
                uint8_t* hi_p = AOP + slot * 2 * TC_A_BLOCK;
#pragma unroll
                for (int i = 0; i < NQ; ++i) {
                    const uint32_t off = (uint32_t)(i * LT + lt) * 16u;
                    const float4 x = make_float4(sv[i].x * ev[i].x, sv[i].y * ev[i].y, sv[i].z * ev[i].z, sv[i].w * ev[i].w);
                    float4 hi, lo;
                    split_tf32_trunc(x, hi, lo);
                    *reinterpret_cast<float4*>(hi_p + off) = hi;
                    *reinterpret_cast<float4*>(hi_p + TC_A_BLOCK + off) = lo;
                }
                fence_proxy_async_smem();
                __syncwarp();
                if (lane == 0) mbar_arrive(&bars->a_full[slot]);
                if (dbg && lane == 0 && warp == F2_TMA_WARP + 1 && q / KBH < 8) g_bwd_dbg[2][q / KBH][(q % KBH) * 3 + 2] = clock64();
            }
        }
    }

    tc_fence_before_sync();
    __syncthreads();
    if (dbg && lane == 0 && warp == 0) g_bwd_dbg[1][7][7] = clock64();
    if (warp == FW_MMA_WARP) {
        tc_fence_after_sync();
        tmem_dealloc(tmem_base, 128);
    }
}

}
namespace {

struct BwdTcArgs {
    const float* gE_next;
    const int32_t* slot;
    const float* gsum;
    int64_t ld_gsum;
    int col_off;
    const float* E_out;
    const float* S;
    const float* E;
    int64_t n_rows;
    int d_in, d_out;
    const float* W1;
    const float* W2;
    float slope;
    const float* mess_mult;
    const uint32_t* mess_bits;
    float mess_p;
    uint64_t seed;
    const uint64_t* seed_dev;
    int layer;
    float* gS;
    float* gEl;
    float* gM;
    float* gb1;
    float* gb2;
    int n_tiles;
    int64_t row_off;
    int d_out_full, out_off, d_in_full, in_off, accumulate, first_in;
    int pf;
};

struct BwdBars {
    uint64_t full_gm, empty_gm, tmem_full[2], tmem_empty[2];
    uint32_t tmem_base;
    float colsum[64];
};

__device__ __forceinline__ uint32_t es_off(int r, int c) { return (uint32_t)r * 256u + (uint32_t)((c ^ (r & 15)) << 4); }

template <int MM, bool PRE>
__global__ void __launch_bounds__(TC_THREADS, 1) dense_bwd_tc_kernel(BwdTcArgs a) {
    extern __shared__ uint8_t smem_raw[];
    const uint32_t base = (smem_u32(smem_raw) + 1023u) & ~1023u;
    uint8_t* smem = smem_raw + (base - smem_u32(smem_raw));
    constexpr int d_in = 64;
    const int d_out = a.d_out;
    const int KBo = d_out / 32;
    uint8_t* GM_hi = smem;
    uint8_t* GM_lo = GM_hi + KBo * TC_A_BLOCK;
    uint8_t* BT_hi = GM_lo + KBo * TC_A_BLOCK;
    uint8_t* BT_lo = BT_hi + KBo * TC_A_BLOCK;
    uint8_t* E_s = BT_lo + KBo * TC_A_BLOCK;
    uint8_t* S_s = E_s + TC_ROWS * 256;
    BwdBars* bars = reinterpret_cast<BwdBars*>(S_s + TC_ROWS * 256);

    const int tid = threadIdx.x, warp = tid >> 5, lane = tid & 31;
    pdl_launch_dependents();

    if (tid == 0) {
        mbar_init(&bars->full_gm, TC_LOAD_WARPS);
        mbar_init(&bars->empty_gm, 1);
        for (int i = 0; i < 2; ++i) {
            mbar_init(&bars->tmem_full[i], 1);
            mbar_init(&bars->tmem_empty[i], TC_EPI_WARPS);
        }
        fence_mbar_init();
    }
    if (warp == TC_EPI_WARPS) tmem_alloc(&bars->tmem_base, 256);
    if (tid < 64) bars->colsum[tid] = 0.f;
    auto prefetch_tile = [&](int tile, bool fwd_tensors, bool grad) {
        const int64_t row0 = (int64_t)tile * TC_ROWS;
        if (row0 >= a.n_rows) return;
        const int64_t nr = a.n_rows - row0 < TC_ROWS ? a.n_rows - row0 : TC_ROWS;
        if (fwd_tensors) {
            l2_prefetch_bulk(a.E_out + row0 * a.d_out_full, (uint32_t)(nr * a.d_out_full * 4));
            l2_prefetch_bulk(a.S + row0 * a.d_in_full, (uint32_t)(nr * a.d_in_full * 4));
            l2_prefetch_bulk(a.E + row0 * a.d_in_full, (uint32_t)(nr * a.d_in_full * 4));
        }
        if (grad && a.gE_next) l2_prefetch_bulk(a.gE_next + row0 * a.d_out_full, (uint32_t)(nr * a.d_out_full * 4));
    };
    if (a.pf > 0 && warp == TC_EPI_WARPS + 1 && lane == 0) {
        for (int i = 0; i < a.pf; ++i) {
            const int tile = blockIdx.x + i * gridDim.x;
            if (tile < a.n_tiles) prefetch_tile(tile, true, false);
        }
    }
    for (int i = tid; i < 128 * KBo * 8; i += TC_THREADS) {
        const int n = i & 127, c = (i >> 7) & 7, kb = i >> 10;
        const float* W = (n < d_in ? a.W1 : a.W2) + a.in_off + (n & 63);
        const int o0 = a.out_off + kb * 32 + c * 4;
        const int64_t ldw = a.d_in_full;
        float4 w = make_float4(W[(int64_t)o0 * ldw], W[(int64_t)(o0 + 1) * ldw], W[(int64_t)(o0 + 2) * ldw],
                               W[(int64_t)(o0 + 3) * ldw]);
        float4 hi, lo;
        split_tf32(w, hi, lo);
        const uint32_t off = kb * TC_A_BLOCK + sw128_offset(n, c);
        *reinterpret_cast<float4*>(BT_hi + off) = hi;
        *reinterpret_cast<float4*>(BT_lo + off) = lo;
    }
    fence_proxy_async_smem();
    tc_fence_before_sync();
    __syncthreads();
    tc_fence_after_sync();
    pdl_wait();
    const uint32_t tmem_base = bars->tmem_base;
    const int n_my = (a.n_tiles - (int)blockIdx.x + (int)gridDim.x - 1) / (int)gridDim.x;
    const bool dbg = g_bwd_dbg_on == 1 && blockIdx.x == 0 && (warp == 0 || warp == TC_EPI_WARPS || warp == TC_EPI_WARPS + 1);
    if (dbg && lane == 0 && warp == 0) g_bwd_dbg[0][7][7] = clock64();

    if (warp < TC_EPI_WARPS) {
        const int r = warp * 32 + lane;
        uint8_t* e_row = E_s + r * 256;
        uint8_t* s_row = S_s + r * 256;
        const int sw = r & 15;
        const int c = lane & 15, hsel = lane >> 4;
        const uint32_t e_s32 = smem_u32(E_s), s_s32 = smem_u32(S_s);
        auto fill = [&](int tile) {
            const int64_t row0 = (int64_t)tile * TC_ROWS;
#pragma unroll 4
            for (int i = 0; i < 16; ++i) {
                const int rl = warp * 32 + 2 * i + hsel;
                const int64_t row = row0 + rl;
                const bool ok = row < a.n_rows;
                const int64_t src = (ok ? row : 0) * a.d_in_full + a.in_off + c * 4;
                const uint32_t off = es_off(rl, c);
                cp_async16(e_s32 + off, a.E + src, ok ? 16u : 0u);
                cp_async16(s_s32 + off, a.S + src, ok ? 16u : 0u);
            }
        };
        if (n_my > 0) fill(blockIdx.x);
        for (int it = 0; it < n_my; ++it) {
            const int tile = blockIdx.x + it * gridDim.x;
            const int buf = it & 1;
            BWD_STAMP(0, it, 0);
            cp_async_wait_all();
            __syncwarp();
            BWD_STAMP(0, it, 1);
            mbar_wait(&bars->tmem_full[buf], (it >> 1) & 1);
            BWD_STAMP(0, it, 2);
            tc_fence_after_sync();
            const uint32_t taddr = tmem_base + ((uint32_t)(warp * 32) << 16) + buf * 128;
#pragma unroll 1
            for (int half = 0; half < d_in / 32; ++half) {
                float v1[32], v2[32];
                tmem_ld_32x32(taddr + half * 32, v1);
                tmem_ld_32x32(taddr + d_in + half * 32, v2);
                if (half == d_in / 32 - 1) {
                    tc_fence_before_sync();
                    __syncwarp();
                    if (lane == 0) mbar_arrive(&bars->tmem_empty[buf]);
                }
#pragma unroll
                for (int j = 0; j < 8; ++j) {
                    const uint32_t off = (uint32_t)(((half * 8 + j) ^ sw) << 4);
                    const float4 e = *reinterpret_cast<const float4*>(e_row + off);
                    const float4 s = *reinterpret_cast<const float4*>(s_row + off);
                    *reinterpret_cast<float4*>(e_row + off) =
                        make_float4(fmaf(v2[4 * j], e.x, v1[4 * j]), fmaf(v2[4 * j + 1], e.y, v1[4 * j + 1]),
                                    fmaf(v2[4 * j + 2], e.z, v1[4 * j + 2]), fmaf(v2[4 * j + 3], e.w, v1[4 * j + 3]));
                    *reinterpret_cast<float4*>(s_row + off) =
                        make_float4(fmaf(v2[4 * j], s.x, v1[4 * j]), fmaf(v2[4 * j + 1], s.y, v1[4 * j + 1]),
                                    fmaf(v2[4 * j + 2], s.z, v1[4 * j + 2]), fmaf(v2[4 * j + 3], s.w, v1[4 * j + 3]));
                }
            }
            __syncwarp();
            BWD_STAMP(0, it, 3);
            const int64_t row0 = (int64_t)tile * TC_ROWS;
#pragma unroll 4
            for (int i = 0; i < 16; ++i) {
                const int rl = warp * 32 + 2 * i + hsel;
                const int64_t row = row0 + rl;
                const uint32_t off = es_off(rl, c);
                float4 x = *reinterpret_cast<const float4*>(E_s + off);
                float4 y = *reinterpret_cast<const float4*>(S_s + off);
                if (row < a.n_rows) {
                    float* ps = a.gS + row * a.d_in_full + a.in_off + c * 4;
                    float* pe = a.gEl + row * a.d_in_full + a.in_off + c * 4;
                    if (a.accumulate) {
                        const float4 x0 = ld_f4(ps), y0 = ld_f4(pe);
                        x.x += x0.x; x.y += x0.y; x.z += x0.z; x.w += x0.w;
                        y.x += y0.x; y.y += y0.y; y.z += y0.z; y.w += y0.w;
                    }
                    st_f4(ps, x);
                    st_f4(pe, y);
                }
            }
            __syncwarp();
            BWD_STAMP(0, it, 4);
            if (it + 1 < n_my) fill(tile + gridDim.x);
        }
    } else if (warp == TC_EPI_WARPS) {
        const uint32_t idesc1 = umma_idesc_tf32(TC_ROWS, 2 * d_in, 0, 0);
        if (a.pf > 0 && lane == 0)
            for (int i = 0; i < a.pf && i < n_my; ++i) prefetch_tile(blockIdx.x + i * gridDim.x, false, true);
        for (int it = 0; it < n_my; ++it) {
            const int buf = it & 1;
            BWD_STAMP(1, it, 0);
            if (a.pf > 0 && lane == 0 && it + a.pf < n_my) prefetch_tile(blockIdx.x + (it + a.pf) * gridDim.x, true, true);
            mbar_wait(&bars->full_gm, it & 1);
            BWD_STAMP(1, it, 1);
            mbar_wait(&bars->tmem_empty[buf], ((it >> 1) & 1) ^ 1);
            BWD_STAMP(1, it, 2);
            tc_fence_after_sync();
            if (lane == 0) {
                const uint32_t tmem_t = tmem_base + buf * 128;
                const uint32_t gm_hi = smem_u32(GM_hi), gm_lo = smem_u32(GM_lo);
                uint32_t acc1 = 0;
                for (int kb = 0; kb < KBo; ++kb) {
#pragma unroll
                    for (int k = 0; k < 4; ++k) {
                        const uint32_t off = kb * TC_A_BLOCK + k * 32;
                        const uint64_t dah = umma_desc_sw128(gm_hi + off, 16, 1024);
                        const uint64_t dal = umma_desc_sw128(gm_lo + off, 16, 1024);
                        const uint64_t dbh = umma_desc_sw128(smem_u32(BT_hi) + off, 16, 1024);
                        const uint64_t dbl = umma_desc_sw128(smem_u32(BT_lo) + off, 16, 1024);
                        umma_tf32(tmem_t, dah, dbh, idesc1, acc1);
                        umma_tf32(tmem_t, dal, dbh, idesc1, 1);
                        umma_tf32(tmem_t, dah, dbl, idesc1, 1);
                        acc1 = 1;
                    }
                }
                umma_commit(&bars->tmem_full[buf]);
                umma_commit(&bars->empty_gm);
            }
            __syncwarp();
            BWD_STAMP(1, it, 3);
        }
    } else {
        const int lw = warp - (TC_EPI_WARPS + 1);
        const int hl = lane & 15, hsel = lane >> 4;
        const int c0 = hl * 4;
        const bool col_ok = c0 < d_out;
        const uint64_t seed = MM == MM_HASH ? ngcf_seed(a.seed, a.seed_dev) : 0ull;
        const uint32_t thr = ngcf_threshold16(a.mess_p);
        const float inv_keep = 1.0f / (1.0f - a.mess_p);
        float4 colsum = make_float4(0.f, 0.f, 0.f, 0.f);
        constexpr int HP = TC_ROWS / (4 * TC_LOAD_WARPS);
        struct Half {
            float4 e[HP], gn[HP];
            int sl[HP];
        };
        auto issue = [&](Half& h, int tile, int half) {
            const int64_t row0 = (int64_t)tile * TC_ROWS;
#pragma unroll
            for (int j = 0; j < HP; ++j) {
                const int64_t row = row0 + 2 * (lw + TC_LOAD_WARPS * (half * HP + j)) + hsel;
                const bool ok = row < a.n_rows && col_ok;
                h.e[j] = h.gn[j] = make_float4(0.f, 0.f, 0.f, 0.f);
                h.sl[j] = -1;
                if (ok) {
                    h.e[j] = ld_stream_f4(a.E_out + row * a.d_out_full + a.out_off + c0);
                    if (a.gE_next) h.gn[j] = ld_stream_f4(a.gE_next + row * a.d_out_full + a.out_off + c0);
                    if (a.slot) h.sl[j] = a.slot[row];
                }
            }
        };
        auto compute = [&](Half& h, int tile, int half) {
            const int64_t row0 = (int64_t)tile * TC_ROWS;
            if (PRE) {
#pragma unroll
                for (int j = 0; j < HP; ++j) {
                    const int s = h.sl[j];
                    if (s >= 0) {
                        const float* gp = a.gsum + (int64_t)s * a.ld_gsum + a.col_off + a.out_off + c0;
                        h.gn[j].x += gp[0]; h.gn[j].y += gp[1]; h.gn[j].z += gp[2]; h.gn[j].w += gp[3];
                    }
                }
            } else {
#pragma unroll
                for (int j = 0; j < HP; ++j) {
                    const int s = h.sl[j];
                    if (__any_sync(FULL_MASK, s >= 0)) {
                        float4 gh = make_float4(0.f, 0.f, 0.f, 0.f);
                        if (s >= 0) {
                            const float* gp = a.gsum + (int64_t)s * a.ld_gsum + a.col_off + a.out_off + c0;
                            gh = make_float4(gp[0], gp[1], gp[2], gp[3]);
                        }
                        const float4 e = h.e[j];
                        float nrm2 = e.x * e.x + e.y * e.y + e.z * e.z + e.w * e.w;
                        float dot = e.x * gh.x + e.y * gh.y + e.z * gh.z + e.w * gh.w;
#pragma unroll
                        for (int o = 8; o > 0; o >>= 1) {
                            nrm2 += __shfl_xor_sync(FULL_MASK, nrm2, o);
                            dot += __shfl_xor_sync(FULL_MASK, dot, o);
                        }
                        if (s >= 0) {
                            const float rn = 1.0f / fmaxf(sqrtf(nrm2), 1e-12f);
                            const float hd = dot * rn;
                            h.gn[j].x += (gh.x - (e.x * rn) * hd) * rn;
                            h.gn[j].y += (gh.y - (e.y * rn) * hd) * rn;
                            h.gn[j].z += (gh.z - (e.z * rn) * hd) * rn;
                            h.gn[j].w += (gh.w - (e.w * rn) * hd) * rn;
                        }
                    }
                }
            }
#pragma unroll
            for (int j = 0; j < HP; ++j) {
                const int r = 2 * (lw + TC_LOAD_WARPS * (half * HP + j)) + hsel;
                const int64_t row = row0 + r;
                const bool in = row < a.n_rows && col_ok;
                const float4 e = h.e[j];
                float4 g = h.gn[j];
                float4 mult = make_float4(1.f, 1.f, 1.f, 1.f);
                if (MM == MM_MULT) {
                    if (in) mult = ld_f4(a.mess_mult + row * a.d_out_full + a.out_off + c0);
                } else if (MM == MM_BITS) {
                    uint32_t w = 0;
                    if (in) w = a.mess_bits[row * ((a.d_out_full + 31) >> 5) + ((a.out_off + c0) >> 5)] >> ((a.out_off + c0) & 31);
                    mult = make_float4(w & 1u ? inv_keep : 0.f, w & 2u ? inv_keep : 0.f, w & 4u ? inv_keep : 0.f,
                                       w & 8u ? inv_keep : 0.f);
                } else if (MM == MM_HASH) {
                    mult = mess_multiplier4_pre(thr, inv_keep, seed, a.layer,
                                                (uint64_t)((row + a.row_off) * a.d_out_full + a.out_off + c0) >> 2);
                }
                g.x *= mult.x * (e.x > 0.f ? 1.f : a.slope);
                g.y *= mult.y * (e.y > 0.f ? 1.f : a.slope);
                g.z *= mult.z * (e.z > 0.f ? 1.f : a.slope);
                g.w *= mult.w * (e.w > 0.f ? 1.f : a.slope);
                if (!in) g = make_float4(0.f, 0.f, 0.f, 0.f);
                if (in && a.first_in) st_f4(a.gM + row * a.d_out_full + a.out_off + c0, g);
                colsum.x += g.x; colsum.y += g.y; colsum.z += g.z; colsum.w += g.w;
                if (col_ok) {
                    float4 hi, lo;
                    split_tf32_trunc(g, hi, lo);
                    const uint32_t off = (hl >> 3) * TC_A_BLOCK + sw128_offset(r, hl & 7);
                    *reinterpret_cast<float4*>(GM_hi + off) = hi;
                    *reinterpret_cast<float4*>(GM_lo + off) = lo;
                }
            }
        };
        Half h0, h1;
        if (n_my > 0) issue(h0, blockIdx.x, 0);
        for (int it = 0; it < n_my; ++it) {
            const int tile = blockIdx.x + it * gridDim.x;
            BWD_STAMP(2, it, 0);
            issue(h1, tile, 1);
            BWD_STAMP(2, it, 1);
            mbar_wait(&bars->empty_gm, (it & 1) ^ 1);
            BWD_STAMP(2, it, 2);
            compute(h0, tile, 0);
            BWD_STAMP(3, it, 0);
            if (it + 1 < n_my) issue(h0, tile + gridDim.x, 0);
            BWD_STAMP(3, it, 1);
            compute(h1, tile, 1);
            BWD_STAMP(3, it, 2);
            fence_proxy_async_smem();
            BWD_STAMP(3, it, 3);
            __syncwarp();
            if (lane == 0) mbar_arrive(&bars->full_gm);
            BWD_STAMP(2, it, 3);
        }
        colsum.x += __shfl_xor_sync(FULL_MASK, colsum.x, 16);
        colsum.y += __shfl_xor_sync(FULL_MASK, colsum.y, 16);
        colsum.z += __shfl_xor_sync(FULL_MASK, colsum.z, 16);
        colsum.w += __shfl_xor_sync(FULL_MASK, colsum.w, 16);
        if (hsel == 0 && col_ok) {
            atomicAdd(&bars->colsum[c0 + 0], colsum.x);
            atomicAdd(&bars->colsum[c0 + 1], colsum.y);
            atomicAdd(&bars->colsum[c0 + 2], colsum.z);
            atomicAdd(&bars->colsum[c0 + 3], colsum.w);
        }
        asm volatile("bar.sync 1, %0;" ::"n"(TC_LOAD_WARPS * 32) : "memory");
        const int lt = tid - (TC_EPI_WARPS + 1) * 32;
        if (lt < d_out && a.first_in) {
            const float cs = bars->colsum[lt];
            atomicAdd(a.gb2 + a.out_off + lt, cs);
            atomicAdd(a.gb1 + a.out_off + lt, 2.0f * cs);
        }
    }

    tc_fence_before_sync();
    __syncthreads();
    if (dbg && lane == 0 && warp == 0) g_bwd_dbg[1][7][7] = clock64();
    if (warp == TC_EPI_WARPS) {
        tc_fence_after_sync();
        tmem_dealloc(tmem_base, 256);
    }
}

constexpr int WG_ROWS = 64;
constexpr int WG_BLOCK = WG_ROWS * 128;

struct WgradArgs {
    const float* S;
    const float* E;
    const float* gM;
    int64_t n_rows;
    int d_out;
    float* gW1;
    float* gW2;
    int n_chunks;
    int d_in_full, in_off, d_out_full, out_off;
    int pf;
};

struct WgBars {
    uint64_t full[2], empty[2], d_full;
    uint32_t tmem_base;
};

__global__ void __launch_bounds__(TC_THREADS, 1) wgrad_tc_kernel(WgradArgs a) {
    extern __shared__ uint8_t smem_raw[];
    const uint32_t base = (smem_u32(smem_raw) + 1023u) & ~1023u;
    uint8_t* smem = smem_raw + (base - smem_u32(smem_raw));
    constexpr int d_in = 64;
    const int d_out = a.d_out;
    const int KBo = d_out / 32;
    const int stage_bytes = (8 + 2 * KBo) * WG_BLOCK;
    WgBars* bars = reinterpret_cast<WgBars*>(smem + 2 * stage_bytes);
    const int tid = threadIdx.x, warp = tid >> 5, lane = tid & 31;
    pdl_launch_dependents();

    if (tid == 0) {
        for (int i = 0; i < 2; ++i) {
            mbar_init(&bars->full[i], TC_LOAD_WARPS);
            mbar_init(&bars->empty[i], 1);
        }
        mbar_init(&bars->d_full, 1);
        fence_mbar_init();
    }
    if (warp == TC_EPI_WARPS) tmem_alloc(&bars->tmem_base, 64);
    tc_fence_before_sync();
    __syncthreads();
    tc_fence_after_sync();
    pdl_wait();
    const uint32_t tmem_d = bars->tmem_base;
    const int n_my = (a.n_chunks - (int)blockIdx.x + (int)gridDim.x - 1) / (int)gridDim.x;
    const bool dbg = g_bwd_dbg_on == 2 && blockIdx.x == 0 && (warp == 0 || warp == TC_EPI_WARPS || warp == TC_EPI_WARPS + 1);
    if (dbg && lane == 0 && warp == 0) g_bwd_dbg[0][7][7] = clock64();

    if (warp < TC_EPI_WARPS) {
        if (a.pf && warp == 0 && lane == 0) {
            for (int it = 0; it < n_my; ++it) {
                const int64_t row0 = (int64_t)(blockIdx.x + it * gridDim.x) * WG_ROWS;
                if (row0 >= a.n_rows) break;
                const int64_t nr = a.n_rows - row0 < WG_ROWS ? a.n_rows - row0 : WG_ROWS;
                l2_prefetch_bulk(a.gM + row0 * a.d_out_full, (uint32_t)(nr * a.d_out_full * 4));
                l2_prefetch_bulk(a.S + row0 * a.d_in_full, (uint32_t)(nr * a.d_in_full * 4));
                l2_prefetch_bulk(a.E + row0 * a.d_in_full, (uint32_t)(nr * a.d_in_full * 4));
            }
        }
        mbar_wait(&bars->d_full, 0);
        BWD_STAMP(0, 0, 0);
        tc_fence_after_sync();
        const int m = warp * 32 + lane;
        float* gw = (m < d_in ? a.gW1 : a.gW2) + (int64_t)a.out_off * a.d_in_full + a.in_off + (m & 63);
        for (int c = 0; c < KBo; ++c) {
            float v[32];
            tmem_ld_32x32(tmem_d + ((uint32_t)(warp * 32) << 16) + c * 32, v);
#pragma unroll
            for (int j = 0; j < 32; ++j) atomicAdd(gw + (int64_t)(c * 32 + j) * a.d_in_full, v[j]);
        }
        BWD_STAMP(0, 0, 1);
    } else if (warp == TC_EPI_WARPS) {
        const uint32_t idesc = umma_idesc_tf32(TC_ROWS, d_out, 1, 1);
        constexpr uint32_t layout = UMMA_SW128_BASE32B, sbo = 512;
        uint32_t acc = 0;
        for (int it = 0; it < n_my; ++it) {
            const int sgi = it & 1;
            mbar_wait(&bars->full[sgi], (it >> 1) & 1);
            tc_fence_after_sync();
            if (lane == 0) {
                const uint32_t x_hi = smem_u32(smem + sgi * stage_bytes), x_lo = x_hi + 4 * WG_BLOCK;
                const uint32_t g_hi = x_lo + 4 * WG_BLOCK, g_lo = g_hi + KBo * WG_BLOCK;
#pragma unroll
                for (int kk = 0; kk < WG_ROWS / 8; ++kk) {
                    const uint32_t off = kk * 1024;
                    const uint64_t dah = umma_desc(x_hi + off, WG_BLOCK, sbo, layout);
                    const uint64_t dal = umma_desc(x_lo + off, WG_BLOCK, sbo, layout);
                    const uint64_t dbh = umma_desc(g_hi + off, WG_BLOCK, sbo, layout);
                    const uint64_t dbl = umma_desc(g_lo + off, WG_BLOCK, sbo, layout);
                    umma_tf32(tmem_d, dah, dbh, idesc, acc);
                    umma_tf32(tmem_d, dal, dbh, idesc, 1);
                    umma_tf32(tmem_d, dah, dbl, idesc, 1);
                    acc = 1;
                }
                umma_commit(&bars->empty[sgi]);
            }
            __syncwarp();
        }
        if (lane == 0) umma_commit(&bars->d_full);
        __syncwarp();
    } else {
        const int lt = tid - (TC_EPI_WARPS + 1) * 32;
        constexpr int LT = TC_LOAD_WARPS * 32;
        const int gq = d_out / 4;
        struct Half {
            float4 s[2], e[2], g[2];
        };
        const int total = 2 * n_my;
        auto issue = [&](Half& h, int i) {
            const int64_t row0 = (int64_t)(blockIdx.x + (i >> 1) * gridDim.x) * WG_ROWS;
#pragma unroll
            for (int q2 = 0; q2 < 2; ++q2) {
                const int idx = ((i & 1) * 2 + q2) * LT + lt, r = idx >> 4, c = idx & 15;
                const int64_t row = row0 + r;
                h.s[q2] = h.e[q2] = h.g[q2] = make_float4(0.f, 0.f, 0.f, 0.f);
                if (row < a.n_rows) {
                    h.s[q2] = ld_stream_f4(a.S + row * a.d_in_full + a.in_off + c * 4);
                    h.e[q2] = ld_stream_f4(a.E + row * a.d_in_full + a.in_off + c * 4);
                    if (c < gq) h.g[q2] = ld_stream_f4(a.gM + row * a.d_out_full + a.out_off + c * 4);
                }
            }
        };
        auto convert = [&](const Half& h, int i) {
            const int sgi = (i >> 1) & 1;
            uint8_t* x_hi = smem + sgi * stage_bytes;
            uint8_t* x_lo = x_hi + 4 * WG_BLOCK;
            uint8_t* g_hi = x_lo + 4 * WG_BLOCK;
            uint8_t* g_lo = g_hi + KBo * WG_BLOCK;
#pragma unroll
            for (int q2 = 0; q2 < 2; ++q2) {
                const int idx = ((i & 1) * 2 + q2) * LT + lt, r = idx >> 4, c = idx & 15;
                const uint32_t off = (c >> 3) * WG_BLOCK + sw128b32_offset(r, c & 7);
                const float4 sv = h.s[q2], ev = h.e[q2];
                const float4 x1 = make_float4(sv.x + ev.x, sv.y + ev.y, sv.z + ev.z, sv.w + ev.w);
                const float4 x2 = make_float4(sv.x * ev.x, sv.y * ev.y, sv.z * ev.z, sv.w * ev.w);
                float4 hi, lo;
                split_tf32(x1, hi, lo);
                *reinterpret_cast<float4*>(x_hi + off) = hi;
                *reinterpret_cast<float4*>(x_lo + off) = lo;
                split_tf32(x2, hi, lo);
                *reinterpret_cast<float4*>(x_hi + 2 * WG_BLOCK + off) = hi;
                *reinterpret_cast<float4*>(x_lo + 2 * WG_BLOCK + off) = lo;
                if (c < gq) {
                    split_tf32(h.g[q2], hi, lo);
                    *reinterpret_cast<float4*>(g_hi + off) = hi;
                    *reinterpret_cast<float4*>(g_lo + off) = lo;
                }
            }
        };
        Half h0, h1;
        if (total > 0) issue(h0, 0);
        for (int i = 0; i < total; i += 2) {
            const int it = i >> 1, sgi = it & 1;
            issue(h1, i + 1);
            mbar_wait(&bars->empty[sgi], ((it >> 1) & 1) ^ 1);
            convert(h0, i);
            if (i + 2 < total) issue(h0, i + 2);
            convert(h1, i + 1);
            fence_proxy_async_smem();
            __syncwarp();
            if (lane == 0) mbar_arrive(&bars->full[sgi]);
            BWD_STAMP(2, it, 0);
        }
    }

    tc_fence_before_sync();
    __syncthreads();
    if (dbg && lane == 0 && warp == 0) g_bwd_dbg[1][7][7] = clock64();
    if (warp == TC_EPI_WARPS) {
        tc_fence_after_sync();
        tmem_dealloc(tmem_d, 64);
    }
}

}

bool ngcf_dense_fwd_tc_eligible(int d_in, int d_out) {
    const bool in_ok = d_in == 32 || d_in == 64 || d_in == 128;
    const bool out_ok = (d_out >= 16 && d_out <= 64 && d_out % 16 == 0) || d_out == 128;
    return in_ok && out_ok;
}

int ngcf_dense_fwd_tc(const float* S, const float* E, int64_t n_rows, int d_in, int d_out, const float* wcat,
                      const float* bias_eff, float slope, const float* mess_mult, const uint32_t* mess_bits, float mess_p,
                      uint64_t seed, const uint64_t* seed_dev, int layer, int64_t row_offset, float* E_out,
                      cudaStream_t st) {
    static bool attr_set_dev[64] = {};
    int cur_dev = 0;
    NGCF_CUDA(cudaGetDevice(&cur_dev));
    bool& attr_set = attr_set_dev[cur_dev & 63];
    if (!attr_set) {
        NGCF_CUDA(cudaFuncSetAttribute(dense_fwd_tma_kernel<MM_NONE>, cudaFuncAttributeMaxDynamicSharedMemorySize, 227 * 1024));
        NGCF_CUDA(cudaFuncSetAttribute(dense_fwd_tma_kernel<MM_MULT>, cudaFuncAttributeMaxDynamicSharedMemorySize, 227 * 1024));
        NGCF_CUDA(cudaFuncSetAttribute(dense_fwd_tma_kernel<MM_BITS>, cudaFuncAttributeMaxDynamicSharedMemorySize, 227 * 1024));
        NGCF_CUDA(cudaFuncSetAttribute(dense_fwd_tma_kernel<MM_HASH>, cudaFuncAttributeMaxDynamicSharedMemorySize, 227 * 1024));
        attr_set = true;
    }
    const int bk = d_in > 64 ? 64 : d_in, bn = d_out > 64 ? 64 : d_out;
    const int KH = d_in / bk, NH = d_out / bn;
    const int n_tiles = (int)ceil_div64(n_rows, TC_ROWS);
    const int grid = (int)min((int64_t)n_tiles, (int64_t)ngcf_num_sms());
    const int KB = 2 * bk / 32;
    const size_t smem = 1024 + (size_t)F2_RAW_STAGES * F2_RAW_BYTES + (size_t)F2_A_SLOTS * 2 * TC_A_BLOCK +
                        (size_t)KB * 2 * bn * 128 + 64 * sizeof(float) + FW_EPI_WARPS * 32 * 32 * sizeof(float) +
                        sizeof(Bars2);
    FwdTmaArgs p{};
    int rc = ngcf_encode_tmap_2d(&p.tmS, S, (uint64_t)n_rows, (uint64_t)d_in, (uint64_t)d_in, 32, TC_ROWS,
                                 CU_TENSOR_MAP_SWIZZLE_128B);
    if (rc == 0)
        rc = ngcf_encode_tmap_2d(&p.tmE, E, (uint64_t)n_rows, (uint64_t)d_in, (uint64_t)d_in, 32, TC_ROWS,
                                 CU_TENSOR_MAP_SWIZZLE_128B);
    NGCF_REQUIRE(rc == 0, "dense_fwd: cuTensorMapEncodeTiled failed (%d)", rc);
    for (int nh = 0; nh < NH; ++nh)
        for (int kh = 0; kh < KH; ++kh) {
            FwdTcArgs a{S, E, n_rows, bk, bn, wcat, bias_eff, slope, mess_mult, mess_bits, mess_p, seed, seed_dev, layer,
                        E_out, n_tiles, row_offset};
            a.ld_in = d_in; a.in_off = kh * bk;
            a.w_row1 = kh * bk; a.w_row2 = d_in + kh * bk;
            a.out_off = nh * bn; a.d_out_full = d_out;
            a.mode = KH == 1 ? FW_SINGLE : (kh == 0 ? FW_PARTIAL : FW_FINAL);
            const int mm = a.mode == FW_PARTIAL ? MM_NONE : mess_mode(mess_mult, mess_bits, mess_p);
            p.b = a;
            switch (mm) {
                case MM_NONE: NGCF_CUDA(ngcf_launch_pdl(dense_fwd_tma_kernel<MM_NONE>, dim3(grid), dim3(F2_THREADS), smem, st, p)); break;
                case MM_MULT: NGCF_CUDA(ngcf_launch_pdl(dense_fwd_tma_kernel<MM_MULT>, dim3(grid), dim3(F2_THREADS), smem, st, p)); break;
                case MM_BITS: NGCF_CUDA(ngcf_launch_pdl(dense_fwd_tma_kernel<MM_BITS>, dim3(grid), dim3(F2_THREADS), smem, st, p)); break;
                default: NGCF_CUDA(ngcf_launch_pdl(dense_fwd_tma_kernel<MM_HASH>, dim3(grid), dim3(F2_THREADS), smem, st, p)); break;
            }
            NGCF_LAUNCH_OK("dense_fwd_tma_kernel");
        }
    return NGCF_OK;
}

static thread_local cudaStream_t g_wgrad_stream = nullptr;
static thread_local int g_wgrad_forked = 0;
extern "C" int ngcf_set_wgrad_stream(void* stream_or_null) {
    g_wgrad_stream = as_stream(stream_or_null);
    return NGCF_OK;
}
extern "C" int ngcf_wgrad_stream_forked(void) {
    const int v = g_wgrad_forked;
    g_wgrad_forked = 0;
    return v;
}

static int dense_prefetch_tiles() {
    static int v = -1;
    if (v < 0) {
        const char* e = getenv("NGCF_B200_PREFETCH");
        v = e ? atoi(e) : 0;
        if (v < 0) v = 0;
        if (v > 8) v = 8;
    }
    return v;
}

bool ngcf_dense_bwd_tc_eligible(int d_in, int d_out, int gh_normalized) {
    if (d_in == 64 && (d_out == 32 || d_out == 64)) return true;
    return (d_in == 64 || d_in == 128) && (d_out == 64 || d_out == 128) && (d_out <= 64 || gh_normalized);
}

int ngcf_dense_bwd_tc(const float* gE_next, const int32_t* slot, const float* gsum, int64_t ld_gsum, int col_off,
                      const float* E_out, const float* S, const float* E, int64_t n_rows, int d_in, int d_out,
                      const float* W1, const float* W2, float slope, const float* mess_mult, const uint32_t* mess_bits,
                      float mess_p, uint64_t seed, const uint64_t* seed_dev, int layer, int64_t row_offset,
                      int gh_normalized, float* gS, float* gEl, float* gW1, float* gb1, float* gW2, float* gb2,
                      float* gM_scratch, cudaStream_t st) {
    const int bn = d_out > 64 ? 64 : d_out;
    const int IH = d_in / 64, OH = d_out / bn;
    const int KBo = bn / 32;
    const int n_tiles = (int)ceil_div64(n_rows, TC_ROWS);
    const size_t smem = 1024 + (size_t)4 * KBo * TC_A_BLOCK + 2 * TC_ROWS * 256 + sizeof(BwdBars);
    const int grid = (int)min((int64_t)n_tiles, (int64_t)ngcf_num_sms());
    void (*kern)(BwdTcArgs) = nullptr;
    const bool pre = gh_normalized != 0;
    switch (mess_mode(mess_mult, mess_bits, mess_p)) {
        case MM_NONE: kern = pre ? dense_bwd_tc_kernel<MM_NONE, true> : dense_bwd_tc_kernel<MM_NONE, false>; break;
        case MM_MULT: kern = pre ? dense_bwd_tc_kernel<MM_MULT, true> : dense_bwd_tc_kernel<MM_MULT, false>; break;
        case MM_BITS: kern = pre ? dense_bwd_tc_kernel<MM_BITS, true> : dense_bwd_tc_kernel<MM_BITS, false>; break;
        default: kern = pre ? dense_bwd_tc_kernel<MM_HASH, true> : dense_bwd_tc_kernel<MM_HASH, false>; break;
    }
    NGCF_CUDA(cudaFuncSetAttribute(kern, cudaFuncAttributeMaxDynamicSharedMemorySize, 227 * 1024));
    NGCF_CUDA(cudaFuncSetAttribute(wgrad_tc_kernel, cudaFuncAttributeMaxDynamicSharedMemorySize, 227 * 1024));
    for (int ih = 0; ih < IH; ++ih)
        for (int oh = 0; oh < OH; ++oh) {
            BwdTcArgs a{gE_next, slot, gsum, ld_gsum, col_off, E_out, S, E, n_rows, 64, bn, W1, W2, slope, mess_mult,
                        mess_bits, mess_p, seed, seed_dev, layer, gS, gEl, gM_scratch, gb1, gb2, n_tiles, row_offset};
            a.d_out_full = d_out; a.out_off = oh * bn; a.d_in_full = d_in; a.in_off = ih * 64;
            a.accumulate = oh > 0; a.first_in = ih == 0;
            const bool contiguous = d_out == bn && d_in == 64 && ((uintptr_t)E_out & 15) == 0 && ((uintptr_t)S & 15) == 0 &&
                                    ((uintptr_t)E & 15) == 0 && ((uintptr_t)gE_next & 15) == 0 && bn % 4 == 0;
            a.pf = contiguous ? dense_prefetch_tiles() : 0;
            NGCF_CUDA(ngcf_launch_pdl(kern, dim3(grid), dim3(TC_THREADS), smem, st, a));
            NGCF_LAUNCH_OK("dense_bwd_tc_kernel");
        }
    const int n_chunks = (int)ceil_div64(n_rows, WG_ROWS);
    const size_t smem2 = 1024 + (size_t)2 * (8 + 2 * KBo) * WG_BLOCK + sizeof(WgBars);
    const int grid2 = (int)min((int64_t)n_chunks, (int64_t)ngcf_num_sms());
    cudaStream_t ws = st;
    if (g_wgrad_stream && g_wgrad_stream != st) {
        static cudaEvent_t ev[64] = {};
        int dev = 0;
        NGCF_CUDA(cudaGetDevice(&dev));
        if (!ev[dev & 63]) NGCF_CUDA(cudaEventCreateWithFlags(&ev[dev & 63], cudaEventDisableTiming));
        NGCF_CUDA(cudaEventRecord(ev[dev & 63], st));
        NGCF_CUDA(cudaStreamWaitEvent(g_wgrad_stream, ev[dev & 63], 0));
        ws = g_wgrad_stream;
        g_wgrad_forked = 1;
    }
    for (int ih = 0; ih < IH; ++ih)
        for (int oh = 0; oh < OH; ++oh) {
            WgradArgs w{S, E, gM_scratch, n_rows, bn, gW1, gW2, n_chunks, d_in, ih * 64, d_out, oh * bn, 0};
            w.pf = (d_out == bn && d_in == 64 && ((uintptr_t)S & 15) == 0 && ((uintptr_t)E & 15) == 0 &&
                    ((uintptr_t)gM_scratch & 15) == 0 && bn % 4 == 0) ? dense_prefetch_tiles() : 0;
            NGCF_CUDA(ngcf_launch_pdl(wgrad_tc_kernel, dim3(grid2), dim3(TC_THREADS), smem2, ws, w));
            NGCF_LAUNCH_OK("wgrad_tc_kernel");
        }
    return NGCF_OK;
}

extern "C" int ngcf_debug_bwd_timeline(int enable, long long* out_host ) {
    NGCF_CUDA(cudaMemcpyToSymbol(g_bwd_dbg_on, &enable, sizeof(int)));
    if (out_host) NGCF_CUDA(cudaMemcpyFromSymbol(out_host, g_bwd_dbg, sizeof(long long) * 4 * 8 * 8));
    return NGCF_OK;
}
```

Measured before the change: 0.4923.

## Store packed activation/dropout codes in forward, read them in backward

The forward tensor-core dense kernel now packs each element's LeakyReLU sign and message-dropout keep bit into a compact code array. The backward kernel gets a new MM_CODES variant that reads these 8-bit-per-float4 codes instead of re-reading the fp32 E_out tile and re-hashing dropout multipliers. This cuts backward memory traffic and hash recomputation. In exchange, forward does extra shared-memory packing and global stores, and every call site carries a new API and checks.

```diff
diff --git a/include/ngcf_b200.h b/include/ngcf_b200.h
--- a/include/ngcf_b200.h
+++ b/include/ngcf_b200.h
@@ -106,6 +106,12 @@
                    const float* wcat, const float* bias_eff, float slope,
                    const float* mess_mult, const uint32_t* mess_bits, float mess_p, uint64_t seed,
                    const uint64_t* seed_dev, int layer, int64_t row_offset, float* E_out, void* stream);
+int ngcf_dense_fwd_codes(const float* S, const float* E, int64_t n_rows, int d_in, int d_out,
+                         const float* wcat, const float* bias_eff, float slope,
+                         const float* mess_mult, const uint32_t* mess_bits, float mess_p, uint64_t seed,
+                         const uint64_t* seed_dev, int layer, int64_t row_offset, float* E_out, void* stream,
+                         uint32_t* act_codes);
+int ngcf_dense_act_code_words(int d_in, int d_out);
 
 int ngcf_mess_dropout_bits(int64_t n_rows, int d_out, float mess_p, uint64_t seed, const uint64_t* seed_dev, int layer,
                            int64_t row_offset, uint32_t* bits, void* stream);
@@ -139,6 +145,13 @@
                    const float* mess_mult, const uint32_t* mess_bits, float mess_p, uint64_t seed,
                    const uint64_t* seed_dev, int layer, int64_t row_offset, int gh_normalized, float* gS, float* gEl,
                    float* gW1, float* gb1, float* gW2, float* gb2, float* gM_scratch, void* stream);
+int ngcf_dense_bwd_codes(const float* gE_next, const int32_t* slot, const float* gsum, int64_t ld_gsum, int col_off,
+                         const float* E_out, const float* S, const float* E, int64_t n_rows, int d_in, int d_out,
+                         const float* W1, const float* W2, float slope,
+                         const float* mess_mult, const uint32_t* mess_bits, float mess_p, uint64_t seed,
+                         const uint64_t* seed_dev, int layer, int64_t row_offset, int gh_normalized, float* gS,
+                         float* gEl, float* gW1, float* gb1, float* gW2, float* gb2, float* gM_scratch, void* stream,
+                         const uint32_t* act_codes);
 
 int ngcf_score_topk_workspace(int64_t n_users, int64_t n_items, int D, int k, size_t* bytes_host);
 int ngcf_score_topk(const float* U, int64_t n_users, const float* I, int64_t n_items, int D, int k,
diff --git a/seoul_tourism_recommendation_ngcf_b200/NGCF.py b/seoul_tourism_recommendation_ngcf_b200/NGCF.py
--- a/seoul_tourism_recommendation_ngcf_b200/NGCF.py
+++ b/seoul_tourism_recommendation_ngcf_b200/NGCF.py
@@ -22,7 +22,7 @@
 
 class _Ctx:
     __slots__ = ("plan", "E", "S", "dims", "vals_f", "vals_b", "mess_mult", "mess_p", "seed", "seed_dev", "masked", "drop_p", "bits_f", "bits_b", "comp_f", "comp_b", "mess_bits",
-                 "rows", "offsets", "W1", "W2", "fresh_key", "node_mode", "last_partial", "fm_stream")
+                 "rows", "offsets", "W1", "W2", "fresh_key", "node_mode", "last_partial", "fm_stream", "grad", "codes")
 
 
 def _capturing() -> bool:
@@ -82,6 +82,7 @@
                                              _lib.int_array(st.dims[:K]), _lib.int_array(st.dims[1:]), K,
                                              _lib.ptr_array(wcats), _lib.ptr_array(biases), _stream()), "pack_weights_all")
         _join_feature_mix(st)
+        st.codes = [None] * K
         for k in range(K):
             d_in, d_out = st.dims[k], st.dims[k + 1]
             vals = st.vals_f[k] if st.vals_f is not None else None
@@ -102,10 +103,13 @@
                     torch.empty(nloc, d_out, dtype=torch.float32, device=dev)
             mm = st.mess_mult[k] if st.mess_mult is not None else None
             E_loc = st.E[k][r0:r0 + nloc]
-            _lib.check(lib.ngcf_dense_fwd(S.data_ptr(), E_loc.data_ptr(), nv, d_in, d_out, wcat.data_ptr(),
-                                          bias.data_ptr(), LEAKY_SLOPE, _lib.ptr(mm[r0:r0 + nloc] if mm is not None else None),
-                                          _lib.ptr(st.mess_bits[k]), float(st.mess_p[k]), st.seed, _lib.ptr(st.seed_dev), k, r0, En.data_ptr(),
-                                          _stream()),
+            words = lib.ngcf_dense_act_code_words(d_in, d_out) if st.grad and mm is None and st.mess_bits[k] is None else 0
+            if words:
+                st.codes[k] = torch.empty(nloc * words, dtype=torch.int32, device=dev)
+            _lib.check(lib.ngcf_dense_fwd_codes(S.data_ptr(), E_loc.data_ptr(), nv, d_in, d_out, wcat.data_ptr(),
+                                                bias.data_ptr(), LEAKY_SLOPE, _lib.ptr(mm[r0:r0 + nloc] if mm is not None else None),
+                                                _lib.ptr(st.mess_bits[k]), float(st.mess_p[k]), st.seed, _lib.ptr(st.seed_dev), k, r0,
+                                                En.data_ptr(), _stream(), _lib.ptr(st.codes[k])),
                        "dense_fwd")
             if xkey is not None and k == K - 1:
                 mod._xchg.push_selected(xkey, r0, nloc, st.rows[:n_sets], st.offsets[:n_sets])
@@ -199,7 +203,7 @@
             if overlap:
                 gM_scratch = torch.empty(nloc, dims[k + 1], dtype=torch.float32, device=dev)
                 gM_keep.append(gM_scratch)
-            _lib.check(lib.ngcf_dense_bwd(_lib.ptr(gE_next), slot_loc.data_ptr(), gsum.data_ptr(), D, col_off,
+            _lib.check(lib.ngcf_dense_bwd_codes(_lib.ptr(gE_next), slot_loc.data_ptr(), gsum.data_ptr(), D, col_off,
                                           st.E[k + 1][r0:r0 + nloc].data_ptr(), st.S[k].data_ptr(),
                                           st.E[k][r0:r0 + nloc].data_ptr(), nv, d_in, d_out,
                                           st.W1[k].data_ptr(), st.W2[k].data_ptr(), LEAKY_SLOPE,
@@ -208,7 +212,7 @@
                                           _lib.ptr(st.seed_dev), k, r0, 1, gS.data_ptr(),
                                           gEl.data_ptr(),
                                           gW1[k].data_ptr(), gb1[k].data_ptr(), gW2[k].data_ptr(), gb2[k].data_ptr(),
-                                          gM_scratch.data_ptr(), _stream()), "dense_bwd")
+                                          gM_scratch.data_ptr(), _stream(), _lib.ptr(st.codes[k])), "dense_bwd")
             if peer:
                 mod._xchg.push(("gS", d_in), r0, nloc)
             elif sh is not None:
@@ -495,6 +499,7 @@
             st.vals_f = [plan.entries(plan.fwd, masks[k]) for k in range(K)]
             st.vals_b = [plan.entries(plan.bwd, masks[k]) for k in range(K)]
         st.rows = [u_id, pos_item] + ([neg_item] if has_neg else [])
+        st.grad = torch.is_grad_enabled() and any(t.requires_grad for t in self.parameters())
         st.offsets = [0, self.n_user] + ([self.n_user] if has_neg else [])
 
         wb = [l.weight for l in self.w1_list] + [l.bias for l in self.w1_list] + \
diff --git a/seoul_tourism_recommendation_ngcf_b200/_lib.py b/seoul_tourism_recommendation_ngcf_b200/_lib.py
--- a/seoul_tourism_recommendation_ngcf_b200/_lib.py
+++ b/seoul_tourism_recommendation_ngcf_b200/_lib.py
@@ -43,6 +43,9 @@
                               C.POINTER(C.c_int), C.c_int, C.POINTER(_vp), C.POINTER(_vp), _vp],
     "ngcf_dense_fwd": [_vp, _vp, _i64, C.c_int, C.c_int, _vp, _vp, _f32, _vp, _vp, _f32, _u64, _vp, C.c_int, _i64, _vp,
                        _vp],
+    "ngcf_dense_fwd_codes": [_vp, _vp, _i64, C.c_int, C.c_int, _vp, _vp, _f32, _vp, _vp, _f32, _u64, _vp, C.c_int, _i64,
+                             _vp, _vp, _vp],
+    "ngcf_dense_act_code_words": [C.c_int, C.c_int],
     "ngcf_mess_dropout_bits": [_i64, C.c_int, _f32, _u64, _vp, C.c_int, _i64, _vp, _vp],
     "ngcf_gather_concat": [C.POINTER(_vp), C.POINTER(C.c_int), C.c_int, _vp, _i64, _i64, _vp, _i64, _vp],
     "ngcf_gather_concat_sets": [C.POINTER(_vp), C.POINTER(C.c_int), C.c_int, C.POINTER(_vp), C.POINTER(_i64), C.POINTER(_i64),
@@ -53,6 +56,8 @@
     "ngcf_rowgrad_reset": [C.POINTER(_vp), C.POINTER(_i64), C.POINTER(_i64), C.c_int, _vp, _vp],
     "ngcf_dense_bwd": [_vp, _vp, _vp, _i64, C.c_int, _vp, _vp, _vp, _i64, C.c_int, C.c_int, _vp, _vp, _f32, _vp, _vp, _f32,
                        _u64, _vp, C.c_int, _i64, C.c_int, _vp, _vp, _vp, _vp, _vp, _vp, _vp, _vp],
+    "ngcf_dense_bwd_codes": [_vp, _vp, _vp, _i64, C.c_int, _vp, _vp, _vp, _i64, C.c_int, C.c_int, _vp, _vp, _f32, _vp, _vp,
+                             _f32, _u64, _vp, C.c_int, _i64, C.c_int, _vp, _vp, _vp, _vp, _vp, _vp, _vp, _vp, _vp],
     "ngcf_set_wgrad_stream": [_vp],
     "ngcf_wgrad_stream_forked": [],
     "ngcf_rowgrad_normalize": [C.POINTER(_vp), C.POINTER(_i64), C.POINTER(_i64), C.c_int, C.POINTER(_vp),
diff --git a/seoul_tourism_recommendation_ngcf_b200/csrc/dense.cu b/seoul_tourism_recommendation_ngcf_b200/csrc/dense.cu
--- a/seoul_tourism_recommendation_ngcf_b200/csrc/dense.cu
+++ b/seoul_tourism_recommendation_ngcf_b200/csrc/dense.cu
@@ -436,7 +436,8 @@
 int ngcf_dense_fwd_tc(const float* S, const float* E, int64_t n_rows, int d_in, int d_out, const float* wcat,
                       const float* bias_eff, float slope, const float* mess_mult, const uint32_t* mess_bits, float mess_p,
                       uint64_t seed,
-                      const uint64_t* seed_dev, int layer, int64_t row_offset, float* E_out, cudaStream_t st);
+                      const uint64_t* seed_dev, int layer, int64_t row_offset, float* E_out, uint32_t* act_codes,
+                      cudaStream_t st);
 
 bool ngcf_dense_bwd_tc_eligible(int d_in, int d_out, int gh_normalized);
 int ngcf_dense_bwd_tc(const float* gE_next, const int32_t* slot, const float* gsum, int64_t ld_gsum, int col_off,
@@ -444,7 +445,13 @@
                       const float* W1, const float* W2, float slope, const float* mess_mult, const uint32_t* mess_bits,
                       float mess_p,
                       uint64_t seed, const uint64_t* seed_dev, int layer, int64_t row_offset, int gh_normalized, float* gS, float* gEl,
-                      float* gW1, float* gb1, float* gW2, float* gb2, float* gM_scratch, cudaStream_t st);
+                      float* gW1, float* gb1, float* gW2, float* gb2, float* gM_scratch, const uint32_t* act_codes,
+                      cudaStream_t st);
+
+extern "C" int ngcf_dense_act_code_words(int d_in, int d_out) {
+    return ngcf_dense_fwd_tc_eligible(d_in, d_out) && ngcf_dense_bwd_tc_eligible(d_in, d_out, 1) ? 2 * ((d_out + 31) / 32)
+                                                                                                 : 0;
+}
 
 extern "C" int ngcf_pack_weights(const float* W1, const float* b1, const float* W2, const float* b2, int d_in,
                                  int d_out, float* wcat, float* bias_eff, void* stream) {
@@ -480,16 +487,28 @@
                               const float* bias_eff, float slope, const float* mess_mult, const uint32_t* mess_bits, float mess_p,
                       uint64_t seed,
                               const uint64_t* seed_dev, int layer, int64_t row_offset, float* E_out, void* stream) {
+    return ngcf_dense_fwd_codes(S, E, n_rows, d_in, d_out, wcat, bias_eff, slope, mess_mult, mess_bits, mess_p, seed,
+                                seed_dev, layer, row_offset, E_out, stream, nullptr);
+}
+
+extern "C" int ngcf_dense_fwd_codes(const float* S, const float* E, int64_t n_rows, int d_in, int d_out,
+                                    const float* wcat, const float* bias_eff, float slope, const float* mess_mult,
+                                    const uint32_t* mess_bits, float mess_p, uint64_t seed, const uint64_t* seed_dev,
+                                    int layer, int64_t row_offset, float* E_out, void* stream, uint32_t* act_codes) {
     NGCF_REQUIRE(S && E && wcat && bias_eff && E_out, "dense_fwd: null pointer");
     NGCF_REQUIRE(d_in > 0 && d_in <= NGCF_MAX_WIDTH && d_out > 0 && d_out <= NGCF_MAX_WIDTH,
                  "dense_fwd: widths %d -> %d not in [1,%d]", d_in, d_out, NGCF_MAX_WIDTH);
     NGCF_REQUIRE(mess_p >= 0.f && mess_p < 1.f, "dense_fwd: mess_p %f not in [0,1)", mess_p);
     NGCF_REQUIRE(n_rows >= 0 && n_rows < ((int64_t)1 << 31), "dense_fwd: n_rows %lld", (long long)n_rows);
+    const bool tc = ngcf_dense_fwd_tc_eligible(d_in, d_out) && aligned16(S) && aligned16(E) && aligned16(E_out) &&
+                    (!mess_mult || aligned16(mess_mult));
+    NGCF_REQUIRE(!act_codes || (tc && !mess_mult && !mess_bits),
+                 "dense_fwd: act_codes need the tensor-core path (widths %d -> %d, 16-byte aligned S / E / E_out) and "
+                 "no mess_mult / mess_bits", d_in, d_out);
     if (n_rows == 0) return NGCF_OK;
-    if (ngcf_dense_fwd_tc_eligible(d_in, d_out) && aligned16(S) && aligned16(E) &&
-        aligned16(E_out) && (!mess_mult || aligned16(mess_mult)))
+    if (tc)
         return ngcf_dense_fwd_tc(S, E, n_rows, d_in, d_out, wcat, bias_eff, slope, mess_mult, mess_bits, mess_p, seed, seed_dev,
-                                 layer, row_offset, E_out, as_stream(stream));
+                                 layer, row_offset, E_out, act_codes, as_stream(stream));
     FwdArgs a{S, E, n_rows, d_in, d_out, wcat, bias_eff, slope, mess_mult, mess_bits, mess_p, seed, seed_dev, layer, E_out,
               (2 * d_in + 3) & ~3, (int)ceil_div64(n_rows, FWD_R), row_offset};
     const int ncg = d_out <= 64 ? 1 : 2;
@@ -514,18 +533,34 @@
                               const float* mess_mult, const uint32_t* mess_bits, float mess_p, uint64_t seed,
                               const uint64_t* seed_dev, int layer, int64_t row_offset, int gh_normalized, float* gS,
                               float* gEl, float* gW1, float* gb1, float* gW2, float* gb2, float* gM_scratch, void* stream) {
+    return ngcf_dense_bwd_codes(gE_next, slot, gsum, ld_gsum, col_off, E_out, S, E, n_rows, d_in, d_out, W1, W2, slope,
+                                mess_mult, mess_bits, mess_p, seed, seed_dev, layer, row_offset, gh_normalized, gS, gEl,
+                                gW1, gb1, gW2, gb2, gM_scratch, stream, nullptr);
+}
+
+extern "C" int ngcf_dense_bwd_codes(const float* gE_next, const int32_t* slot, const float* gsum, int64_t ld_gsum,
+                                    int col_off, const float* E_out, const float* S, const float* E, int64_t n_rows,
+                                    int d_in, int d_out, const float* W1, const float* W2, float slope,
+                                    const float* mess_mult, const uint32_t* mess_bits, float mess_p, uint64_t seed,
+                                    const uint64_t* seed_dev, int layer, int64_t row_offset, int gh_normalized,
+                                    float* gS, float* gEl, float* gW1, float* gb1, float* gW2, float* gb2,
+                                    float* gM_scratch, void* stream, const uint32_t* act_codes) {
     NGCF_REQUIRE(E_out && S && E && W1 && W2 && gS && gEl && gW1 && gb1 && gW2 && gb2, "dense_bwd: null pointer");
     NGCF_REQUIRE(!slot || gsum, "dense_bwd: slot given without gsum");
     NGCF_REQUIRE(d_in > 0 && d_in <= NGCF_MAX_WIDTH && d_out > 0 && d_out <= NGCF_MAX_WIDTH,
                  "dense_bwd: widths %d -> %d not in [1,%d]", d_in, d_out, NGCF_MAX_WIDTH);
     NGCF_REQUIRE(mess_p >= 0.f && mess_p < 1.f, "dense_bwd: mess_p %f not in [0,1)", mess_p);
     NGCF_REQUIRE(n_rows >= 0 && n_rows < ((int64_t)1 << 31), "dense_bwd: n_rows %lld", (long long)n_rows);
+    const bool tc = gM_scratch && ngcf_dense_bwd_tc_eligible(d_in, d_out, gh_normalized) && aligned16(S) &&
+                    aligned16(E) && aligned16(gS) && aligned16(gEl) && aligned16(gM_scratch);
+    NGCF_REQUIRE(!act_codes || (tc && gh_normalized && !mess_mult && !mess_bits),
+                 "dense_bwd: act_codes need the tensor-core path (widths %d -> %d, gM_scratch, 16-byte aligned operands), "
+                 "gh_normalized and no mess_mult / mess_bits", d_in, d_out);
     if (n_rows == 0) return NGCF_OK;
-    if (gM_scratch && ngcf_dense_bwd_tc_eligible(d_in, d_out, gh_normalized) && aligned16(S) &&
-        aligned16(E) && aligned16(gS) && aligned16(gEl) && aligned16(gM_scratch))
+    if (tc)
         return ngcf_dense_bwd_tc(gE_next, slot, gsum, ld_gsum, col_off, E_out, S, E, n_rows, d_in, d_out, W1, W2,
                                  slope, mess_mult, mess_bits, mess_p, seed, seed_dev, layer, row_offset, gh_normalized, gS,
-                                 gEl, gW1, gb1, gW2, gb2, gM_scratch, as_stream(stream));
+                                 gEl, gW1, gb1, gW2, gb2, gM_scratch, act_codes, as_stream(stream));
     BwdArgs a{gE_next, slot, gsum, ld_gsum, col_off, E_out, S, E, n_rows, d_in, d_out, W1, W2, slope, mess_mult,
               mess_bits, mess_p, seed, seed_dev, layer, gS, gEl, gW1, gb1, gW2, gb2, 0, row_offset, gh_normalized};
     int rc;
diff --git a/seoul_tourism_recommendation_ngcf_b200/csrc/dense_tc.cu b/seoul_tourism_recommendation_ngcf_b200/csrc/dense_tc.cu
--- a/seoul_tourism_recommendation_ngcf_b200/csrc/dense_tc.cu
+++ b/seoul_tourism_recommendation_ngcf_b200/csrc/dense_tc.cu
@@ -40,6 +40,7 @@
     int64_t row_off;
     int64_t ld_in;
     int in_off, w_row1, w_row2, out_off, d_out_full, mode;
+    uint32_t* act_codes;
 };
 enum { FW_SINGLE = 0, FW_PARTIAL = 1, FW_FINAL = 2 };
 
@@ -48,7 +49,7 @@
 
 __device__ __forceinline__ int stage_off(int r, int c) { return r * 32 + ((c ^ (r & 7)) << 2); }
 
-enum { MM_NONE = 0, MM_MULT = 1, MM_BITS = 2, MM_HASH = 3 };
+enum { MM_NONE = 0, MM_MULT = 1, MM_BITS = 2, MM_HASH = 3, MM_CODES = 4 };
 static inline int mess_mode(const float* mess_mult, const uint32_t* mess_bits, float mess_p) {
     return mess_mult ? MM_MULT : (mess_p > 0.f ? (mess_bits ? MM_BITS : MM_HASH) : MM_NONE);
 }
@@ -90,6 +91,7 @@
         __syncwarp();
         BWD_STAMP(0, it, 4);
         const int col = c * 32 + c4 * 4;
+        uint32_t code[8] = {};
         if (col < d_out) {
             const int gcol = a.out_off + col;
             const float4 b4 = *reinterpret_cast<const float4*>(bias_s + col);
@@ -113,6 +115,7 @@
                 x.y = x.y > 0.f ? x.y : a.slope * x.y;
                 x.z = x.z > 0.f ? x.z : a.slope * x.z;
                 x.w = x.w > 0.f ? x.w : a.slope * x.w;
+                uint32_t keep = 0xfu;
                 if (MM == MM_BITS) {
                     const uint32_t w = a.mess_bits[row * words + (gcol >> 5)] >> (gcol & 31);
                     x.x = w & 1u ? x.x * inv_keep : 0.f; x.y = w & 2u ? x.y * inv_keep : 0.f;
@@ -121,11 +124,36 @@
                     const float4 mm = mess_multiplier4_pre(thr, inv_keep, seed, a.layer,
                                                            (uint64_t)((row + a.row_off) * a.d_out_full + gcol) >> 2);
                     x.x *= mm.x; x.y *= mm.y; x.z *= mm.z; x.w *= mm.w;
+                    keep = (mm.x != 0.f ? 1u : 0u) | (mm.y != 0.f ? 2u : 0u) | (mm.z != 0.f ? 4u : 0u) |
+                           (mm.w != 0.f ? 8u : 0u);
                 } else if (MM == MM_MULT) {
                     const float4 mm = ld_f4(a.mess_mult + row * a.d_out_full + gcol);
                     x.x *= mm.x; x.y *= mm.y; x.z *= mm.z; x.w *= mm.w;
                 }
+                code[i] = keep | (x.x > 0.f ? 0x10u : 0u) | (x.y > 0.f ? 0x20u : 0u) | (x.z > 0.f ? 0x40u : 0u) |
+                          (x.w > 0.f ? 0x80u : 0u);
                 st_f4(dst, x);
+            }
+        }
+        if (a.act_codes) {
+            uint8_t* cb = reinterpret_cast<uint8_t*>(st);
+#pragma unroll
+            for (int i = 0; i < 8; ++i) cb[(i * 4 + rr) * 8 + c4] = (uint8_t)code[i];
+            __syncwarp();
+            const uint2 raw = *reinterpret_cast<const uint2*>(cb + lane * 8);
+            __syncwarp();
+            const uint64_t u = (uint64_t)raw.x | ((uint64_t)raw.y << 32);
+            auto pack = [](uint64_t v) {
+                v &= 0x0F0F0F0F0F0F0F0Full;
+                v = (v | (v >> 4)) & 0x00FF00FF00FF00FFull;
+                v = (v | (v >> 8)) & 0x0000FFFF0000FFFFull;
+                return (uint32_t)(v | (v >> 16));
+            };
+            const int64_t row = row_base + lane;
+            if (row < a.n_rows) {
+                const int64_t cw = 2 * ((a.d_out_full + 31) >> 5);
+                *reinterpret_cast<uint2*>(a.act_codes + row * cw + 2 * ((a.out_off + c * 32) >> 5)) =
+                    make_uint2(pack(u), pack(u >> 4));
             }
         }
         BWD_STAMP(0, it, 2);
@@ -388,6 +416,7 @@
     int n_tiles;
     int64_t row_off;
     int d_out_full, out_off, d_in_full, in_off, accumulate, first_in;
+    const uint32_t* act_codes;
     int pf;
 };
 
@@ -600,7 +629,10 @@
         struct Half {
             float4 e[HP], gn[HP];
             int sl[HP];
+            uint32_t code[HP];
         };
+        const int64_t code_ld = 2 * ((a.d_out_full + 31) >> 5);
+        const int code_word = 2 * ((a.out_off + c0) >> 5), code_shift = (a.out_off + c0) & 31;
         auto issue = [&](Half& h, int tile, int half) {
             const int64_t row0 = (int64_t)tile * TC_ROWS;
 #pragma unroll
@@ -609,8 +641,14 @@
                 const bool ok = row < a.n_rows && col_ok;
                 h.e[j] = h.gn[j] = make_float4(0.f, 0.f, 0.f, 0.f);
                 h.sl[j] = -1;
+                h.code[j] = 0;
                 if (ok) {
-                    h.e[j] = ld_stream_f4(a.E_out + row * a.d_out_full + a.out_off + c0);
+                    if (MM == MM_CODES) {
+                        const uint2 w = __ldg(reinterpret_cast<const uint2*>(a.act_codes + row * code_ld + code_word));
+                        h.code[j] = ((w.x >> code_shift) & 0xfu) | ((w.y >> code_shift) & 0xfu) << 4;
+                    } else {
+                        h.e[j] = ld_stream_f4(a.E_out + row * a.d_out_full + a.out_off + c0);
+                    }
                     if (a.gE_next) h.gn[j] = ld_stream_f4(a.gE_next + row * a.d_out_full + a.out_off + c0);
                     if (a.slot) h.sl[j] = a.slot[row];
                 }
@@ -675,10 +713,18 @@
                     mult = mess_multiplier4_pre(thr, inv_keep, seed, a.layer,
                                                 (uint64_t)((row + a.row_off) * a.d_out_full + a.out_off + c0) >> 2);
                 }
-                g.x *= mult.x * (e.x > 0.f ? 1.f : a.slope);
-                g.y *= mult.y * (e.y > 0.f ? 1.f : a.slope);
-                g.z *= mult.z * (e.z > 0.f ? 1.f : a.slope);
-                g.w *= mult.w * (e.w > 0.f ? 1.f : a.slope);
+                if (MM == MM_CODES) {
+                    const uint32_t w = h.code[j];
+                    g.x *= (w & 0x01u ? inv_keep : 0.f) * (w & 0x10u ? 1.f : a.slope);
+                    g.y *= (w & 0x02u ? inv_keep : 0.f) * (w & 0x20u ? 1.f : a.slope);
+                    g.z *= (w & 0x04u ? inv_keep : 0.f) * (w & 0x40u ? 1.f : a.slope);
+                    g.w *= (w & 0x08u ? inv_keep : 0.f) * (w & 0x80u ? 1.f : a.slope);
+                } else {
+                    g.x *= mult.x * (e.x > 0.f ? 1.f : a.slope);
+                    g.y *= mult.y * (e.y > 0.f ? 1.f : a.slope);
+                    g.z *= mult.z * (e.z > 0.f ? 1.f : a.slope);
+                    g.w *= mult.w * (e.w > 0.f ? 1.f : a.slope);
+                }
                 if (!in) g = make_float4(0.f, 0.f, 0.f, 0.f);
                 if (in && a.first_in) st_f4(a.gM + row * a.d_out_full + a.out_off + c0, g);
                 colsum.x += g.x; colsum.y += g.y; colsum.z += g.z; colsum.w += g.w;
@@ -928,7 +974,7 @@
 int ngcf_dense_fwd_tc(const float* S, const float* E, int64_t n_rows, int d_in, int d_out, const float* wcat,
                       const float* bias_eff, float slope, const float* mess_mult, const uint32_t* mess_bits, float mess_p,
                       uint64_t seed, const uint64_t* seed_dev, int layer, int64_t row_offset, float* E_out,
-                      cudaStream_t st) {
+                      uint32_t* act_codes, cudaStream_t st) {
     static bool attr_set_dev[64] = {};
     int cur_dev = 0;
     NGCF_CUDA(cudaGetDevice(&cur_dev));
@@ -963,6 +1009,7 @@
             a.w_row1 = kh * bk; a.w_row2 = d_in + kh * bk;
             a.out_off = nh * bn; a.d_out_full = d_out;
             a.mode = KH == 1 ? FW_SINGLE : (kh == 0 ? FW_PARTIAL : FW_FINAL);
+            a.act_codes = a.mode == FW_PARTIAL ? nullptr : act_codes;
             const int mm = a.mode == FW_PARTIAL ? MM_NONE : mess_mode(mess_mult, mess_bits, mess_p);
             p.b = a;
             switch (mm) {
@@ -1009,7 +1056,7 @@
                       const float* W1, const float* W2, float slope, const float* mess_mult, const uint32_t* mess_bits,
                       float mess_p, uint64_t seed, const uint64_t* seed_dev, int layer, int64_t row_offset,
                       int gh_normalized, float* gS, float* gEl, float* gW1, float* gb1, float* gW2, float* gb2,
-                      float* gM_scratch, cudaStream_t st) {
+                      float* gM_scratch, const uint32_t* act_codes, cudaStream_t st) {
     const int bn = d_out > 64 ? 64 : d_out;
     const int IH = d_in / 64, OH = d_out / bn;
     const int KBo = bn / 32;
@@ -1018,7 +1065,8 @@
     const int grid = (int)min((int64_t)n_tiles, (int64_t)ngcf_num_sms());
     void (*kern)(BwdTcArgs) = nullptr;
     const bool pre = gh_normalized != 0;
-    switch (mess_mode(mess_mult, mess_bits, mess_p)) {
+    switch (act_codes ? MM_CODES : mess_mode(mess_mult, mess_bits, mess_p)) {
+        case MM_CODES: kern = dense_bwd_tc_kernel<MM_CODES, true>; break;
         case MM_NONE: kern = pre ? dense_bwd_tc_kernel<MM_NONE, true> : dense_bwd_tc_kernel<MM_NONE, false>; break;
         case MM_MULT: kern = pre ? dense_bwd_tc_kernel<MM_MULT, true> : dense_bwd_tc_kernel<MM_MULT, false>; break;
         case MM_BITS: kern = pre ? dense_bwd_tc_kernel<MM_BITS, true> : dense_bwd_tc_kernel<MM_BITS, false>; break;
@@ -1032,6 +1080,7 @@
                         mess_bits, mess_p, seed, seed_dev, layer, gS, gEl, gM_scratch, gb1, gb2, n_tiles, row_offset};
             a.d_out_full = d_out; a.out_off = oh * bn; a.d_in_full = d_in; a.in_off = ih * 64;
             a.accumulate = oh > 0; a.first_in = ih == 0;
+            a.act_codes = act_codes;
             const bool contiguous = d_out == bn && d_in == 64 && ((uintptr_t)E_out & 15) == 0 && ((uintptr_t)S & 15) == 0 &&
                                     ((uintptr_t)E & 15) == 0 && ((uintptr_t)gE_next & 15) == 0 && bn % 4 == 0;
             a.pf = contiguous ? dense_prefetch_tiles() : 0;
```

Result: slower. 0.5001 (median of 6 runs) (+1.6%).
